# slimgroup/SetIntersectionProjection.jl

Hardware: AMD Instinct MI355X
Metric: PARSDMM iterations/sec (higher is better)
Workload: dtype f32

## Files before the change

### setintersectionprojection.jl_amd/csrc/engine.cpp

```cpp
#include "engine.h"
#include "comm.h"
#include "dist_dft.h"
#include "ext_proj.h"

#include <algorithm>
#include <chrono>
#include <cmath>
#include <cstdio>
#include <cstdlib>
#include <cstring>
#include <limits>
#include <map>
#include <mutex>
#include <thread>
#include <exception>

namespace sipx {

const LaunchObserver*& launch_observer() {
  static thread_local const LaunchObserver* obs = nullptr;
  return obs;
}

namespace {
EnvKnobs g_env_knobs;
}
const EnvKnobs& env_knobs() { return g_env_knobs; }
void refresh_env_knobs() {
  auto num = [](const char* name, long long dflt) { const char* e = std::getenv(name); return e ? std::atoll(e) : dflt; };
  EnvKnobs k;
  k.cds_march = (int)num("SIPX_CDS_MARCH", 1);
  k.cds_march_zchunk = num("SIPX_CDS_MARCH_ZCHUNK", 0);
  k.multi_zchunk = num("SIPX_MULTI_ZCHUNK", 0);
  k.rhs_march = (int)num("SIPX_RHS_MARCH", 1);
  k.rhs_march_zchunk = num("SIPX_RHS_MARCH_ZCHUNK", 0);
  k.q_plan = (int)num("SIPX_Q_PLAN", 1);
  k.mark_stride = (int)std::max<long long>(0, num("SIPX_MARK_STRIDE", 0));
  k.trace_searches = (int)num("SIPX_TRACE_SEARCHES", 0);
  k.trace_kernels = (int)num("SIPX_TRACE_KERNELS", 0);
  g_env_knobs = k;
}
long long*& alloc_tally() {
  static thread_local long long* t = nullptr;
  return t;
}

namespace {

struct TallyGuard {
  long long* prev;
  explicit TallyGuard(long long* t) : prev(alloc_tally()) { alloc_tally() = t; }
  ~TallyGuard() { alloc_tally() = prev; }
};

struct ObserverGuard {
  const LaunchObserver* prev;
  explicit ObserverGuard(const LaunchObserver* o) : prev(launch_observer()) { launch_observer() = o; }
  ~ObserverGuard() { launch_observer() = prev; }
};

constexpr int SLOTS = SET_SLOTS;

inline std::map<void*, long long>& tally_sizes() {
  static std::map<void*, long long> m;
  return m;
}
inline std::mutex& tally_mutex() {
  static std::mutex m;
  return m;
}
inline void tally_add(void* p, long long bytes) {
  if (long long* t = alloc_tally()) {
    *t += bytes;
    std::lock_guard<std::mutex> lk(tally_mutex());
    tally_sizes()[p] += bytes;
  }
}
inline void tally_release(void* p) {
  long long* t = alloc_tally();
  std::lock_guard<std::mutex> lk(tally_mutex());
  auto it = tally_sizes().find(p);
  if (it == tally_sizes().end()) return;
  if (t) *t -= it->second;
  tally_sizes().erase(it);
}
inline std::map<void*, size_t>& alloc_sizes() {
  static std::map<void*, size_t> m;
  return m;
}
template <typename T>
T* dalloc(size_t n, bool zero = true) {
  T* p = nullptr;
  if (n == 0) return p;
  SIPX_HIP(hipMalloc(&p, n * sizeof(T)));
  tally_add(p, (long long)(n * sizeof(T)));
  {
    std::lock_guard<std::mutex> lk(tally_mutex());
    alloc_sizes()[p] = n * sizeof(T);
  }
  if (zero) {
    SIPX_HIP(hipMemset(p, 0, n * sizeof(T)));
    SIPX_HIP(hipStreamSynchronize(nullptr));
  }
  return p;
}
struct SparseBlock {
  size_t total = 0;
  std::vector<std::pair<size_t, size_t>> maps;
  std::vector<hipMemGenericAllocationHandle_t> handles;
};
inline std::map<void*, SparseBlock>& sparse_registry() {
  static std::map<void*, SparseBlock> reg;
  return reg;
}
inline std::mutex& sparse_mutex() {
  static std::mutex m;
  return m;
}
constexpr size_t SPARSE_GRAN = 2ull << 20;
// ... 184 lines not shown
  long long Mtrue = 0, Mpad = 0;
  long long blk_rows[3] = {0, 0, 0};
  T plo = 0, phi = 0;
  bool ident = true, two_pass = false, is_dist = false, owned = true;
  bool in_sweep = false;
  T *y = nullptr, *l = nullptr, *dy = nullptr, *lh0 = nullptr, *y0 = nullptr, *s0 = nullptr, *l0 = nullptr;
  T *y2 = nullptr, *l2 = nullptr;
  int snap = -1;
  T *lb = nullptr, *ub = nullptr, *ata = nullptr;
  std::vector<void*> halo_allocs;
  int searches_done = 0;
  int ext_kind = 0;
  bool dist_ext = false;
  int owner_rank = 0;
  bool slab_ext = false, fan = false, slab_card = false, slab_dft = false;
  std::shared_ptr<DistDft<T>> ddft;
  int fan_owner = 0;
  bool fan_on_side = false;
  T* fanv = nullptr;
  hipEvent_t fan_ev = nullptr;
  ExtSpec spec;
  std::vector<T> host_basis;
  std::shared_ptr<ExtProj<T>> ext;
  ProjScalars<T>* ps = nullptr;
  ProjScalars<T>* psf = nullptr;
  std::vector<long long> ata_off;
  std::vector<T> host_lb, host_ub, host_ata;
  double sums[SLOTS] = {0};
  bool bb_valid = false;
  T last_rho = T(-1), last_gamma = T(-1);
  hipStream_t st = nullptr;
  hipEvent_t ev = nullptr;
  long long cbuf_len = 0;
  double* ptmp = nullptr;
  T *mpart = nullptr, *cbuf = nullptr;
};

}

template <typename T>
class Engine : public EngineBase {
 public:
  Engine(int ndim, const int64_t* n, const double* h, int device) : device_(device) {
    if (ndim != 2 && ndim != 3) throw std::runtime_error("ndim must be 2 or 3");
    SIPX_HIP(hipSetDevice(device));
    SIPX_HIP(hipStreamCreateWithFlags(&stream_, hipStreamNonBlocking));
    SIPX_HIP(hipEventCreateWithFlags(&ev_fork_, hipEventDisableTiming));
    SIPX_HIP(hipEventCreateWithFlags(&ev_fork2_, hipEventDisableTiming));
    {
      const char* e = std::getenv("SIPX_SERIAL_SETS");
      set_streams_ = !(e && e[0] == '1');
      const char* f = std::getenv("SIPX_CDS_FULL");
      cds_full_ = f && f[0] == '1';
      const char* k = std::getenv("SIPX_SET_STREAMS");
      if (k && std::atoi(k) > 0) { n_set_streams_ = std::atoi(k); set_streams_forced_ = true; }
    }
    ndim_ = ndim;
    for (int a = 0; a < 3; ++a) {
      G_.n[a] = a < ndim ? n[a] : 1;
      if (G_.n[a] < 1) throw std::runtime_error("grid size must be positive");
      ih_[a] = a < ndim ? T(1) / T(h[a]) : T(0);
    }
    if (ndim == 3 && G_.n[2] == 1) ndim_ = 2;
    G_.N = G_.n[0] * G_.n[1] * G_.n[2];
    if (G_.N <= (1ll << 22) && !set_streams_forced_ && !std::getenv("SIPX_SERIAL_SETS")) set_streams_ = false;
    G_.st[0] = 1;
    G_.st[1] = G_.n[0];
    G_.st[2] = G_.n[0] * G_.n[1];
    if (G_.N >= (1ll << 31)) throw std::runtime_error("grids of 2^31 points or more are not supported");
    G_.set_fast_div();
  }
  ~Engine() override {
    (void)hipSetDevice(device_);
    if (lane_thr_.joinable()) lane_thr_.join();
    if (lane_st_) { (void)hipStreamSynchronize(lane_st_); (void)hipStreamDestroy(lane_st_); }
    for (hipEvent_t e : {lane_fork_, lane_ev_}) if (e) (void)hipEventDestroy(e);
    dfree(lane_v_);
    if (fan_st_) { (void)hipStreamSynchronize(fan_st_); (void)hipStreamDestroy(fan_st_); }
    if (fan_fork_) (void)hipEventDestroy(fan_fork_);
    for (void* p : {(void*)fan_ptmp_, (void*)fan_mpart_, (void*)fan_c_}) dfree(p);
    if (loose_owned_) { dfree(loose_v_); dfree(loose_w_); }
    (void)hipStreamSynchronize(stream_);
    for (auto& s : sets_) free_set(s);
    for (void* p : {(void*)xr_base_[0], (void*)xr_base_[1], (void*)xr_base_[2], (void*)w_base_, (void*)rhs_, (void*)m_base_, (void*)r_base_, (void*)p_base_, (void*)p2_base_, (void*)Ap_, (void*)Q_, (void*)Q2_,
                    (void*)scr_v_, (void*)scr_c_, (void*)scr_i_, (void*)scr_w_, (void*)part_cg_, (void*)part_tmp_, (void*)part_sets_,
                    (void*)maxpart_, (void*)cg_dev_, (void*)gbuf_, (void*)stage_, (void*)sstage_, (void*)fbuf_, (void*)agree_buf_})
      dfree(p);
    comm_.reset();
    if (cstream_) (void)hipStreamDestroy(cstream_);
    for (auto e : ev_c_) if (e) (void)hipEventDestroy(e);
    if (ev_sums_) (void)hipEventDestroy(ev_sums_);
    for (hipEvent_t e : open_ev_) if (e) (void)hipEventDestroy(e);
    if (ev_cgb_) (void)hipEventDestroy(ev_cgb_);
    if (ticket_) (void)hipHostFree((void*)ticket_);
    if (cg_host_) (void)hipHostFree(cg_host_);
    if (hres_) (void)hipHostFree(hres_);
    if (sums_word_) (void)hipHostFree((void*)sums_word_);
    dfree(sums_ticket_);
    if (hlean_) (void)hipHostFree((void*)hlean_);
    if (hovf_) (void)hipHostFree((void*)hovf_);
    if (hverd_) (void)hipHostFree((void*)hverd_);
    for (auto e : ev_) (void)hipEventDestroy(e);
    for (auto e : stat_ev_) (void)hipEventDestroy(e);
    for (auto e : cg_ev_) if (e) (void)hipEventDestroy(e);
    for (hipStream_t q : pool_) if (q != stream_) (void)hipStreamDestroy(q);
    if (ev_fork_) (void)hipEventDestroy(ev_fork_);
    if (ev_fork2_) (void)hipEventDestroy(ev_fork2_);
    (void)hipStreamDestroy(stream_);
  }

  int add_set(const sipx_set_desc* d, const void* ata_R, const int64_t* ata_off, int d_i) override {
    if (finalized_) throw std::runtime_error("sipx_add_set after sipx_finalize");
    SetState<T> s;
    if (d->op == SIPX_OP_CSC) configure_custom(s, d);
    else configure_op(s, d->op);
    configure_proj(s, d);
    if (s.custom && !ata_R) throw std::runtime_error("a custom sparse operator needs its A'A in CDS (ata_R, ata_off)");
    if (s.custom && (s.comp || s.ext_kind))
      throw std::runtime_error("custom sparse operators: Minkowski components and library-backed projectors are not available");
    if (ata_R && s.comp) throw std::runtime_error("Minkowski sets use descriptor-generated AtA (pass ata_R = NULL)");
    if (ata_R) {
      if (d_i < 1 || d_i > 9) throw std::runtime_error("AtA band count out of range (1..9 bands per set)");
      s.ata_off.assign(ata_off, ata_off + d_i);
      s.host_ata.assign((const T*)ata_R, (const T*)ata_R + (size_t)G_.N * d_i);
    } else {
      s.ata_off = default_ata_offsets(s);
    }
    sets_.push_back(std::move(s));
    return (int)sets_.size() - 1;
  }

  int64_t set_rows(int set) override {
    if (set == (int)sets_.size() && !finalized_) return G_.N;
    if (set < 0 || set >= (int)sets_.size()) throw std::runtime_error("set index out of range");
    return sets_[set].Mtrue;
  }
  void num_terms(int* p, int* pp) override {
    if (p) *p = p_n_;
    if (pp) *pp = pp_n_;
  }
  void set_owned(const int32_t* owned) override {
    if (finalized_) throw std::runtime_error("sipx_set_owned must precede sipx_finalize");
    owned_.assign(owned, owned + sets_.size() + 1);
  }

  void set_decomp(int mode) override {
    if (finalized_) throw std::runtime_error("sipx_set_decomp must precede sipx_finalize");
    if (mode != SIPX_DECOMP_SETS && mode != SIPX_DECOMP_SLAB && mode != SIPX_DECOMP_SLAB_FULL) throw std::runtime_error("unknown decomposition");
    slab_req_ = mode != SIPX_DECOMP_SETS;
    slab_full_req_ = mode == SIPX_DECOMP_SLAB_FULL;
  }

  void set_comm(Comm* c) override {
    std::unique_ptr<Comm> hold(c);
    if (finalized_) throw std::runtime_error("the communicator must be attached before sipx_finalize");
    counting_ = c ? new CountingComm(hold.release()) : nullptr;
    comm_.reset(counting_);
  }
  void comm_info(int* nranks, int* rank, char* version, int version_len, int* decomposition) override {
    if (version && version_len > 0) version[0] = 0;
    if (nranks) *nranks = 1;
    if (rank) *rank = 0;
    if (decomposition) *decomposition = (finalized_ ? slab_ : (slab_req_ && comm_)) ? SIPX_DECOMP_SLAB : SIPX_DECOMP_SETS;
    if (comm_) comm_->info(nranks, rank, version, version_len > 0 ? (size_t)version_len : 0);
    else if (version && version_len > 0) std::snprintf(version, (size_t)version_len, "none");
  }
  void bind_device() override { SIPX_HIP(hipSetDevice(device_)); }
// ... 363 lines not shown
      if (sweep_plain_ && s.in_sweep) { s.y2 = halloc(s.Mpad); s.l2 = halloc(s.Mpad); }
      if (s.custom) upload_custom(s);
      if (s.slab_dft) {
        const long long nn[3] = {G_.n[0], G_.n[1], G_.n[2]};
        s.ddft = std::make_shared<DistDft<T>>(nn, r0_ / plane_, r1_ / plane_, chunk_ / plane_, comm_->world, comm_->rank, (double)s.spec.pmax, stream_);
      }
      if (s.ext_kind && !s.dist_ext && !s.slab_ext && !s.slab_dft && !(s.fan && s.fan_owner != comm_->rank)) {
        s.spec.lb = s.host_lb.empty() ? nullptr : s.host_lb.data();
        s.spec.ub = s.host_ub.empty() ? nullptr : s.host_ub.data();
        s.spec.basis = s.host_basis.empty() ? nullptr : s.host_basis.data();
        s.ext = std::make_shared<ExtProj<T>>(s.spec, stream_);
        if (s.ext_kind == EXT_HISTOGRAM) { s.host_lb.clear(); s.host_ub.clear(); }
        s.host_basis.clear();
        s.host_basis.shrink_to_fit();
      }
      if (s.fan) {
        s.fanv = (s.fan_owner == comm_->rank || !slab_local_) ? dalloc<T>(fullpad) : loose_alloc(Npad);
        SIPX_HIP(hipEventCreateWithFlags(&s.fan_ev, hipEventDisableTiming));
        if (s.fan_owner == comm_->rank && !fan_st_) {
          SIPX_HIP(hipStreamCreateWithFlags(&fan_st_, hipStreamNonBlocking));
          SIPX_HIP(hipEventCreateWithFlags(&fan_fork_, hipEventDisableTiming));
          fan_ptmp_ = dalloc<double>((size_t)(PREP_SLOTS + 2) * NB);
          fan_mpart_ = dalloc<T>(2 * NB);
          fan_c_ = dalloc<T>(fullpad);
        }
      }
      if (s.two_pass) {
        s.ps = dalloc<ProjScalars<T>>(1);
        s.psf = dalloc<ProjScalars<T>>(1);
        K<T>::ps_init(stream_, s.ps, scr_i_);
        K<T>::ps_init(stream_, s.psf, scr_i_);
      }
      if ((slab_ || search_batch_) && s.two_pass) {
        s.ptmp = dalloc<double>((size_t)(PREP_SLOTS + 2) * NB);
        s.mpart = dalloc<T>(2 * NB);
        s.cbuf_len = slab_local_ ? std::min<long long>(s.Mpad, std::max<long long>((long long)s.nblk_or1() * (whi_ - wlo_), hooks_.gcap + 64)) : s.Mpad;
        s.cbuf = dalloc<T>(s.cbuf_len);
      }
      const bool had_scratch = s.ptmp != nullptr;
      if (set_streams_ && !s.ext_kind && s.prox != PX_CARD) {
        if ((int)pool_.size() < n_set_streams_) {
          hipStream_t q = stream_;
          if (!pool_.empty()) SIPX_HIP(hipStreamCreateWithFlags(&q, hipStreamNonBlocking));
          pool_.push_back(q);
        }
        if (search_streams_) {
          while ((int)pool_.size() < n_set_streams_) {
            hipStream_t q2 = stream_;
            if (!pool_.empty()) SIPX_HIP(hipStreamCreateWithFlags(&q2, hipStreamNonBlocking));
            pool_.push_back(q2);
          }
          s.st = s.two_pass ? pool_[(size_t)(++search_next_) % pool_.size()] : pool_[0];
        } else {
          s.st = pool_[pool_next_++ % pool_.size()];
        }
        SIPX_HIP(hipEventCreateWithFlags(&s.ev, hipEventDisableTiming));
        if (s.two_pass && !had_scratch) {
          s.ptmp = dalloc<double>((size_t)(PREP_SLOTS + 2) * NB);
          s.mpart = dalloc<T>(2 * NB);
          s.cbuf = dalloc<T>(s.Mpad);
        }
      }
      if (s.prox == SIPX_PROJ_BOUNDS_VEC) {
        s.lb = dalloc<T>(s.Mpad); s.ub = dalloc<T>(s.Mpad);
        upload_rows(s, s.host_lb.data(), s.lb);
        upload_rows(s, s.host_ub.data(), s.ub);
      }
      if (warm && l0 && l0[i]) upload_rows_ranged(s, (const T*)l0[i], s.l);
      if (warm && y0 && y0[i]) upload_rows_ranged(s, (const T*)y0[i], s.y);
    }
    if (search_batch_) {
      int n2 = 0;
      for (auto& s : sets_) n2 += s.two_pass ? 1 : 0;
      fbuf_ = dalloc<T>((size_t)n2 * fast_hdr<T>());
      stage_ = dalloc<double>((size_t)n2 * (PREP_SLOTS + 1 + 2));
    }
    if (warm && x0) {
      const long long c0 = slab_local_ ? std::max<long long>(0, wlo_) : 0, c1 = slab_local_ ? std::min<long long>(Nx_, whi_) : Nx_;
      if (c1 > c0) SIPX_HIP(hipMemcpy(x_ + c0, (const T*)x0 + c0, (c1 - c0) * sizeof(T), hipMemcpyHostToDevice));
    }

    assemble_Q();
    if (q_fused_ && !stencil_q_ && !comm_ && cds_.march != 0) Q2_ = dalloc<T>((size_t)Nx_ * cds_.d);
    {
      const char* ln = std::getenv("SIPX_RANK_LANE");
      lane_set_ = -1;
      if (!comm_ && !mk_ && sweep_partial_ && !(ln && ln[0] == '0'))
        for (int i = 0; i < p_n_ && lane_set_ < 0; ++i) {
          const SetState<T>& s = sets_[i];
          if (s.owned && !s.in_sweep && !s.dist_ext && s.ident && !s.custom && s.ext && (s.ext_kind == EXT_RANK || s.ext_kind == EXT_NUCLEAR)) lane_set_ = i;
        }
      if (comm_ && slab_ && slab_loose_ && !mk_ && sweep_partial_ && !(ln && ln[0] == '0'))
        for (int i = 0; i < p_n_ && lane_set_ < 0; ++i) {
          const SetState<T>& s = sets_[i];
          if (s.owned && !s.in_sweep && s.slab_ext && s.ident && !s.custom && s.ext && (s.ext_kind == EXT_RANK || s.ext_kind == EXT_NUCLEAR)) lane_set_ = i;
        }
      if (lane_set_ >= 0) {
        const char* lp = std::getenv("SIPX_LANE_PRIORITY");
        int pr_least = 0, pr_greatest = 0;
        SIPX_HIP(hipDeviceGetStreamPriorityRange(&pr_least, &pr_greatest));
        if (lp && lp[0] == '0') SIPX_HIP(hipStreamCreateWithFlags(&lane_st_, hipStreamNonBlocking));
        else SIPX_HIP(hipStreamCreateWithPriority(&lane_st_, hipStreamNonBlocking, lp && lp[0] == 'l' ? pr_least : pr_greatest));
        SIPX_HIP(hipEventCreateWithFlags(&lane_fork_, hipEventDisableTiming));
        SIPX_HIP(hipEventCreateWithFlags(&lane_ev_, hipEventDisableTiming));
        if (slab_) lane_v_ = (slab_local_ && !loose_whole_) ? loose_alloc(Npad) : dalloc<T>((size_t)std::max<long long>(fullpad, sets_[lane_set_].Mpad));
        else lane_v_ = dalloc<T>((size_t)sets_[lane_set_].Mpad);
      }
    }
    } catch (const std::exception& ex) {
      if (!comm_ || comm_->world <= 1 || !agree_buf_) throw;
      alloc_err = ex.what();
    }
    if (comm_ && comm_->world > 1 && agree_buf_) {
      const double flag = alloc_err.empty() ? 0.0 : 1.0;
      double sum = flag;
      try {
        SIPX_HIP(hipMemcpy(agree_buf_, &flag, sizeof(double), hipMemcpyHostToDevice));
        comm_->allreduce_sum(agree_buf_, 1, SIPX_F64, stream_);
        SIPX_HIP(hipStreamSynchronize(stream_));
        SIPX_HIP(hipMemcpy(&sum, agree_buf_, sizeof(double), hipMemcpyDeviceToHost));
      } catch (const std::exception& ex) {
        throw std::runtime_error(std::string("sipx_finalize: the ranks could not agree on the outcome of their allocations (") + ex.what() + ")" +
                                 (alloc_err.empty() ? "" : "; this rank: " + alloc_err));
      }
      if (sum != 0.0)
        throw std::runtime_error("sipx_finalize failed on " + std::to_string((int)sum) + " of " + std::to_string(comm_->world) + " ranks while allocating" +
                                 (alloc_err.empty() ? std::string(" (not on this one)") : ": " + alloc_err));
    }
    finalized_ = true;

    initial_feasibility(feasibility_initial);
  }

  void reset(const void* m, const double* rho_ini, int n_rho, double gamma_ini, int zero_ini_guess, const void* x0,
             const void* const* l0, const void* const* y0, double* feasibility_initial) override {
    need_final();
    if (comm_) throw std::runtime_error("sipx_reset is not available for a rank of a sharded solve (build a new context)");
    SIPX_HIP(hipSetDevice(device_));
    if (lane_thr_.joinable()) lane_thr_.join();
    lane_err_ = nullptr;
    SIPX_HIP(hipStreamSynchronize(stream_));
    for (hipStream_t q : pool_) if (q && q != stream_) SIPX_HIP(hipStreamSynchronize(q));
    if (lane_st_) SIPX_HIP(hipStreamSynchronize(lane_st_));
    if (cstream_) SIPX_HIP(hipStreamSynchronize(cstream_));
    const long long N = G_.N;
    for (int k = 0; k < 3; ++k) dzero(xr_base_[k], stream_);
    dzero(p_base_, stream_); dzero(rhs_, stream_); dzero(r_base_, stream_); dzero(Ap_, stream_);
    dzero(p2_base_, stream_); dzero(w_base_, stream_); dzero(Q2_, stream_);
    dzero(part_cg_, stream_); dzero(part_tmp_, stream_); dzero(part_sets_, stream_); dzero(maxpart_, stream_);
    dzero(cg_dev_, stream_); dzero(sums_ticket_, stream_);
    dzero(fbuf_, stream_); dzero(stage_, stream_); dzero(sstage_, stream_); dzero(gbuf_, stream_);
    dzero(scr_v_, stream_); dzero(scr_c_, stream_); dzero(scr_w_, stream_);
    if (scr_i_) dzero(scr_i_, stream_);
    dzero(lane_v_, stream_);
    SIPX_HIP(hipMemcpyAsync(m_, m, N * sizeof(T), hipMemcpyHostToDevice, stream_));
    x_cur_ = 0; x_snap_ = -1;
    x_ = xr_[0]; xold_ = x_;
    if (n_rho == 1) std::fill(rho_.begin(), rho_.end(), (T)rho_ini[0]);
    else if (n_rho == p_n_) for (int i = 0; i < p_n_; ++i) rho_[i] = (T)rho_ini[i];
    else throw std::runtime_error("rho_ini must have 1 or p entries");
    T g0 = (T)gamma_ini;
    if (any_ncvx_) g0 = T(0.75);
    std::fill(gamma_.begin(), gamma_.end(), g0);
    const bool warm = !zero_ini_guess;
    for (int i = 0; i < p_n_; ++i) {
      SetState<T>& s = sets_[i];
      for (void* b : s.halo_allocs) dzero(b, stream_);
      dzero(s.lh0, stream_); dzero(s.s0, stream_);
      dzero(s.sbuf, stream_);
      dzero(s.ptmp, stream_); dzero(s.mpart, stream_); dzero(s.cbuf, stream_);
      s.snap = -1;
      s.searches_done = 0;
      std::fill(s.sums, s.sums + SLOTS, 0.0);
      s.bb_valid = false;
      s.last_rho = T(-1); s.last_gamma = T(-1);
      if (s.ps) K<T>::ps_init(stream_, s.ps, scr_i_);
      if (s.psf) K<T>::ps_init(stream_, s.psf, scr_i_);
      if (s.ext) { s.ext->set_stream(stream_); s.ext->reset(); }
      if (warm && l0 && l0[i]) upload_rows_ranged(s, (const T*)l0[i], s.l);
      if (warm && y0 && y0[i]) upload_rows_ranged(s, (const T*)y0[i], s.y);
    }
    if (warm && x0) SIPX_HIP(hipMemcpyAsync(x_, x0, Nx_ * sizeof(T), hipMemcpyHostToDevice, stream_));
    std::memset(cg_host_, 0, 2 * sizeof(CgState<T>));
    std::memset((void*)ticket_, 0xff, 64);
    std::memset(hres_, 0, sizeof(double) * (p_n_ + 1) * SLOTS);
    std::memset((void*)sums_word_, 0, 64);
    std::memset((void*)hlean_, 0, sizeof(int) * (p_n_ + 1));
    std::memset((void*)hovf_, 0, sizeof(int) * (p_n_ + 1));
    std::memset((void*)hverd_, 0, sizeof(unsigned) * (p_n_ + 1));
    sums_seq_ = 0; cg_seq_ = 0; spec_seq_ = 0;
    spec_searches_ = spec_fallbacks_ = spec_rounds_ = 0;
    batch_searches_ = batch_fallbacks_ = 0;
    head_done_ = false; rs_pending_ = false; sums_pending_ = false; defer_sums_ = false; merge_sums_ = false; merged_nslots_ = 0;
    q_pending_ = false; q_defer_ = false; rhs_fused_ = false; fuse_rhs_ = false; have_log_sums_ = false;
    obj_ss_ = evo_ss_ = xx_ss_ = 0;
    sums_flags_ = 0; word_sums_ = false;
    for (bool& v : open_valid_) v = false;
    mark_weight_[0] = mark_weight_[1] = 1.0;
    nmark_[0] = nmark_[1] = 0;
    mark_step_[0] = mark_step_[1] = 0;
    run_ = Run();
    assemble_Q();
    initial_feasibility(feasibility_initial);
  }

  void initial_feasibility(double* feasibility_initial) {
    feas_init_.assign(pp_n_, 0.0);
    for (int i = 0; i < pp_n_; ++i) {
      SetState<T>& s = sets_[i];
      if (s.dist_ext || s.slab_ext || s.slab_dft) {
        dist_feasibility(s, m_, part_sets_ + ((size_t)i * SLOTS + SL_FE2) * NB, i);
        continue;
      }
      if (s.fan) {
        SetArgs<T> a = set_args(s, rho_[i], gamma_[i], 0);
        a.x = m_;
        fan_feasibility(s, a, part_sets_ + ((size_t)i * SLOTS + SL_FE2) * NB);
        continue;
      }
      if (!s.owned) continue;
      if (slab_local_ && !s.two_pass && !s.ext_kind && !s.custom) {
        SetArgs<T> a = set_args(s, rho_[i], gamma_[i], 0);
        a.x = m_;
        K<T>::proj_dist_set(stream_, Gr_, a, 1, (const ProjScalars<T>*)nullptr, part_sets_ + ((size_t)i * SLOTS + SL_FE2) * NB);
        continue;
      }
      if (slab_ && !s.two_pass && comm_->rank != 0) continue;
      double* dst = part_sets_ + ((size_t)i * SLOTS + SL_FE2) * NB;
      const T* mm = s.comp == 2 ? w_ : m_;
      if (s.ext_kind) {
        SetArgs<T> a = set_args(s, rho_[i], gamma_[i], 0);
        a.x = mm;
        ext_feasibility(s, a, dst);
      } else if (s.custom) {
        K<T>::csr_spmv(stream_, s.Mtrue, s.d_rowptr, s.d_colidx, s.d_rval, mm, s.sbuf);
        if (s.two_pass) {
          SetArgs<T> a = set_args(s, rho_[i], gamma_[i], 0);
          a.x = s.sbuf;
          K<T>::proj_scalars_set(stream_, s.gm, a, 1, s.psf, part_tmp_, maxpart_, scr_c_, s.Mtrue);
          K<T>::proj_dist_set(stream_, s.gm, a, 1, s.psf, dst);
        } else {
          proj_dist_grid<T>(stream_, s.gm, 0, s.dir, s.Mpad, s.sbuf, s.prox, s.plo, s.phi, s.lb, s.ub, nullptr, dst);
        }
      } else if (s.two_pass) {
        SetArgs<T> a = set_args(s, rho_[i], gamma_[i], 0);
        a.x = mm;
        SampleCtl cf;
        cf.host_ovf = (int*)hovf_ + i;
        cf.compact_cap = scr_c_len_;
        K<T>::proj_scalars_set(stream_, Gr_, a, 1, s.psf, part_tmp_, maxpart_, scr_c_, s.Mtrue, cf, hooks());
        K<T>::proj_dist_set(stream_, Gr_, a, 1, s.psf, dst);
      } else {
        K<T>::fwd(stream_, G_, s.nblk, s.dir, s.ih, mm, scr_v_);
        proj_dist_grid<T>(stream_, G_, s.nblk, s.dir, s.Mpad, scr_v_, s.prox, s.plo, s.phi, s.lb, s.ub, nullptr, dst);
      }
    }
    reduce_set_sums(p_n_ * SLOTS);
    SIPX_HIP(hipStreamSynchronize(stream_));
    for (int i = 0; i < p_n_ && slab_; ++i)
      if (hovf_[i]) {
        hovf_[i] = 0;
        throw std::runtime_error("initial feasibility of set " + std::to_string(i) + ": the magnitudes inside the final bracket of the l1 search, gathered over all ranks, exceed the exchange segment of " +
                                 std::to_string(hooks_.gcap) + " values per rank (slab decomposition) -- use the set decomposition for this problem");
      }
    for (int i = 0; i < pp_n_; ++i) {
      if (!sets_[i].owned && !comm_) continue;
      feas_init_[i] = (double)feas_value(hres_[i * SLOTS + SL_FE2], hres_[i * SLOTS + SL_SS2]);
    }
    if (feasibility_initial)
      for (int i = 0; i < pp_n_; ++i) feasibility_initial[i] = feas_init_[i];
  }

  void rhs_compose(const double* rho) override {
    need_final();
    ObserverGuard og(observer());
    head_done_ = false;
    if (rs_pending_) {
      SIPX_HIP(hipStreamWaitEvent(stream_, ev_c_[1], 0));
      rs_pending_ = false;
    }
    if (mk_) {
      for (int half = 0; half < 2; ++half) {
        T* out = rhs_ + (long long)half * G_.N;
        int launched = 0;
        for (int pass = 0; pass < 2; ++pass) {
// ... 1258 lines not shown
      if (s.is_dist) {
        obj_ss_ = h[SL_OBJ]; evo_ss_ = h[SL_EVO]; xx_ss_ = h[SL_XX];
        if (mk_) { evo_ss_ = hres_[(size_t)p_n_ * SLOTS + SL_EVO]; xx_ss_ = hres_[(size_t)p_n_ * SLOTS + SL_XX]; }
        have_log_sums_ = true;
      }
    }
    if (all && !slab_dist_logs_) {
      const double* g = hres_ + (size_t)p_n_ * SLOTS;
      obj_ss_ = g[SL_OBJ]; evo_ss_ = g[SL_EVO]; xx_ss_ = g[SL_XX];
      have_log_sums_ = true;
    }
    if ((flags & SIPX_YL_FEAS) && feas) {
      for (int i = 0; i < pp_n_; ++i) {
        feas[i] = 0;
        if (!sets_[i].owned && !all) continue;
        const double* h = hres_ + (size_t)i * SLOTS;
        feas[i] = (sets_[i].two_pass || sets_[i].ext_kind) ? (double)feas_value(h[SL_FE2], h[SL_SS2])
                                                            : (double)feas_value(h[SL_FE], h[SL_SS]);
      }
    }
  }

  void log_scalars(double* obj, double* evol_x) override {
    need_final();
    ObserverGuard og(observer());
    if (!have_log_sums_) {
      K<T>::log3(stream_, G_.N, mk_ ? w_ : x_, m_, xold_, part_sets_);
      if (mk_) K<T>::log3(stream_, Nx_, x_, (const T*)nullptr, xold_, part_sets_ + (size_t)SLOTS * NB);
      K<T>::fin_sum(stream_, part_sets_, (mk_ ? 2 : 1) * SLOTS, nullptr, hres_);
      SIPX_HIP(hipStreamSynchronize(stream_));
      obj_ss_ = hres_[SL_OBJ]; evo_ss_ = hres_[SL_EVO]; xx_ss_ = hres_[SL_XX];
      if (mk_) { evo_ss_ = hres_[SLOTS + SL_EVO]; xx_ss_ = hres_[SLOTS + SL_XX]; }
    }
    const T nd = (T)std::sqrt(obj_ss_);
    *obj = (double)(T(0.5) * (nd * nd));
    *evol_x = (double)((T)std::sqrt(evo_ss_) / (T)std::sqrt(xx_ss_));
  }

  void adapt_rho_gamma(int adjust_rho, int adjust_gamma, double* rho_io, double* gamma_io) override {
    need_final();
    for (int i = 0; i < p_n_; ++i) {
      SetState<T>& s = sets_[i];
      if (!s.owned && !comm_) continue;
      if (!s.bb_valid)
        throw std::runtime_error("sipx_adapt_rho_gamma: call sipx_update_y_l with SIPX_YL_BB (or _FIRST) first");
      T rho = (T)rho_io[i], gamma = (T)gamma_io[i];
      const double* h = s.sums;
      bb_rule<T>((T)h[SL_HL], (T)std::sqrt(h[SL_HH]), (T)std::sqrt(h[SL_LH]), (T)std::sqrt(h[SL_DL]),
                 (T)std::sqrt(h[SL_GG]), (T)h[SL_GL], adjust_rho != 0, adjust_gamma != 0, rho, gamma);
      rho_io[i] = (double)rho;
      gamma_io[i] = (double)gamma;
    }
  }

  void q_update(const double* rho_new, const double* rho_old) override {
    need_final();
    ObserverGuard og(observer());
    if (stencil_q_) {
      stencil_weights(rho_new);
      return;
    }
    if (mk_) {
      std::vector<T> al(p_n_);
      for (int i = 0; i < p_n_; ++i) al[i] = rho_new[i] == rho_old[i] ? T(0) : (T)rho_new[i] - (T)rho_old[i];
      mk_q_update(al);
      return;
    }
    flush_q_pending();
    QArgs<T> a;
    a.nsets = 0;
    for (int i = 0; i < p_n_; ++i) {
      if (rho_new[i] == rho_old[i]) continue;
      push_qset(a, sets_[i], (T)rho_new[i] - (T)rho_old[i]);
    }
    if (q_defer_ && q_fused_ && cds_.march != 0 && !comm_ && a.nsets > 0) {
      bool generated = true;
      for (int k = 0; k < a.nsets; ++k) generated &= a.s[k].ata == nullptr;
      if (generated) {
        q_pending_args_ = a;
        q_pending_ = true;
        return;
      }
    }
    K<T>::q_update(stream_, G_, qr0_, qr1_, cds_, a, Q_);
  }
  void flush_q_pending() {
    if (!q_pending_) return;
    q_pending_ = false;
    K<T>::q_update(stream_, G_, qr0_, qr1_, cds_, q_pending_args_, Q_);
  }

  void warm_start_from(EngineBase* coarse_base) override {
    need_final();
    auto* c = dynamic_cast<Engine<T>*>(coarse_base);
    if (!c || !c->finalized_) throw std::runtime_error("warm start: the coarse context must be a finalized context of the same precision");
    if (c->device_ != device_) throw std::runtime_error("warm start: both levels must live on one device");
    if (c->p_n_ != p_n_ || c->ndim_ != ndim_ || mk_ || c->mk_) throw std::runtime_error("warm start: the two levels must hold the same sets");
    if ((comm_ != nullptr) != (c->comm_ != nullptr) || (comm_ && !(slab_ && c->slab_)))
      throw std::runtime_error("warm start between levels of a sharded solve needs both levels slab-decomposed (sipx_set_decomp)");
    long long nc[3], nf[3];
    for (int a = 0; a < 3; ++a) { nc[a] = c->G_.n[a]; nf[a] = G_.n[a]; }
    const long long Nc = c->G_.N, Nf = G_.N;
    const long long cpad = c->comm_ ? c->chunk_ * c->comm_->world : Nc;
    int nbmax = 1;
    for (auto& st : c->sets_) nbmax = std::max(nbmax, st.nblk_or1());
    T* whole = c->slab_ ? dalloc<T>((size_t)nbmax * cpad, false) : nullptr;
    const int dt = dtype_code();
    const long long f0 = slab_local_ ? std::max<long long>(0, wlo_) : 0, f1 = slab_local_ ? std::min<long long>(Nf, whi_) : Nf;
    auto complete = [&](const T* src, int nb) -> const T* {
      if (!c->slab_) return src;
      const long long nloc = c->r1_ - c->r0_;
      for (int q = 0; q < nb; ++q) {
        T* w = whole + (long long)q * cpad;
        if (nloc > 0) SIPX_HIP(hipMemcpyAsync(w + c->r0_, src + (long long)q * Nc + c->r0_, nloc * sizeof(T), hipMemcpyDeviceToDevice, stream_));
        c->comm_->allgather(w, (size_t)c->chunk_, dt, stream_);
      }
      return whole;
    };
    const long long cstride = c->slab_ ? cpad : Nc;
    SIPX_HIP(hipStreamSynchronize(c->stream_));
    resample_nn_padded<T>(stream_, nc, nf, nc, nf, f0, f1, complete(c->x_, 1), x_);
    for (int i = 0; i < p_n_; ++i) {
      SetState<T>&f = sets_[i], &g = c->sets_[i];
      if (f.custom || g.custom || f.nblk != g.nblk) throw std::runtime_error("warm start: operator kinds differ between the levels");
      for (int q = 0; q < f.nblk; ++q)
        if (f.dir[q] != g.dir[q]) throw std::runtime_error("warm start: operator kinds differ between the levels");
      if (!f.owned || !g.owned) continue;
      for (int which = 0; which < 2; ++which) {
        const T* src = complete(which ? g.y : g.l, g.nblk_or1());
        T* dst = which ? f.y : f.l;
        if (f.nblk >= 2) {
          for (int q = 0; q < f.nblk; ++q)
            resample_nn_rows<T>(stream_, nc, nf, f.nblk, f.dir, q, cstride, f0, f1, src, dst + (long long)q * Nf);
        } else {
          long long cc[3], cf[3];
          for (int a = 0; a < 3; ++a) { cc[a] = nc[a]; cf[a] = nf[a]; }
          if (f.nblk == 1) { cc[f.dir[0]] -= 1; cf[f.dir[0]] -= 1; }
          resample_nn_padded<T>(stream_, nc, nf, cc, cf, f0, f1, src, dst);
        }
      }
    }
    SIPX_HIP(hipStreamSynchronize(stream_));
    dfree(whole);
  }

  void gather_slabs(bool want_x, const std::vector<char>& want_l, const std::vector<char>& want_y) {
    const int dt = dtype_code();
    if (want_x) comm_->allgather(x_, (size_t)chunk_, dt, stream_);
    for (int i = 0; i < p_n_; ++i)
      for (int which = 0; which < 2; ++which) {
        if (!(which ? want_y[i] : want_l[i])) continue;
        T* arr = which ? sets_[i].y : sets_[i].l;
        const int nb = sets_[i].nblk > 0 ? sets_[i].nblk : 1;
        for (int q = 0; q < nb; ++q) {
          T* blk = arr + (long long)q * G_.N;
          if (r1_ > r0_) SIPX_HIP(hipMemcpyAsync(scr_v_ + r0_, blk + r0_, (r1_ - r0_) * sizeof(T), hipMemcpyDeviceToDevice, stream_));
          comm_->allgather(scr_v_, (size_t)chunk_, dt, stream_);
          SIPX_HIP(hipMemcpyAsync(blk, scr_v_, G_.N * sizeof(T), hipMemcpyDeviceToDevice, stream_));
        }
      }
  }

  void download_sparse(void* x, void* const* l, void* const* y) {
    const int dt = dtype_code();
    const long long N = G_.N, Npad = chunk_ * comm_->world, nloc = r1_ - r0_;
    int nbmax = 1;
    for (auto& s : sets_) nbmax = std::max(nbmax, s.nblk_or1());
    T* exch = dalloc<T>((size_t)Npad);
    T* whole = dalloc<T>((size_t)nbmax * N);
    auto complete = [&](const T* src) {
      if (nloc > 0) SIPX_HIP(hipMemcpyAsync(exch + r0_, src + r0_, nloc * sizeof(T), hipMemcpyDeviceToDevice, stream_));
      comm_->allgather(exch, (size_t)chunk_, dt, stream_);
// ... 286 lines not shown
    for (int a = 0; a < 3; ++a) H = std::max<long long>(H, G_.st[a]);
    H = (H + 3) / 4 * 4;
    T* dxb = dalloc<T>(G_.N + 2 * H);
    T* dvb = dalloc<T>(s.Mpad + H);
    T *dx = dxb + H, *dv = dvb + H;
    if (!adjoint) {
      SIPX_HIP(hipMemcpy(dx, x, G_.N * sizeof(T), hipMemcpyHostToDevice));
      K<T>::fwd(stream_, G_, s.nblk, s.dir, s.ih, dx, dv);
      download_rows(s, dv, (T*)out);
    } else {
      upload_rows(s, (const T*)x, dv);
      K<T>::adj(stream_, G_, s.nblk, s.dir, s.ih, dv, dx);
      SIPX_HIP(hipStreamSynchronize(stream_));
      SIPX_HIP(hipMemcpy(out, dx, G_.N * sizeof(T), hipMemcpyDeviceToHost));
    }
    dfree(dxb);
    dfree(dvb);
  }

  void project(const sipx_set_desc* d, void* v, int64_t len) override {
    SIPX_HIP(hipSetDevice(device_));
    Grid g1;
    g1.n[0] = len; g1.n[1] = 1; g1.n[2] = 1; g1.N = len; g1.st[0] = 1; g1.st[1] = len; g1.st[2] = len;
    T* dv = dalloc<T>(len);
    T* dc = dalloc<T>(len);
    T *lb = nullptr, *ub = nullptr;
    double* part = dalloc<double>((size_t)(PREP_SLOTS + 2) * NB);
    T* mp = dalloc<T>(2 * NB);
    ProjScalars<T>* ps = dalloc<ProjScalars<T>>(1);
    SIPX_HIP(hipMemcpy(dv, v, len * sizeof(T), hipMemcpyHostToDevice));
    const int prox = d->proj;
    const T plo = (T)d->pmin, phi = (T)d->pmax;
    if (prox == SIPX_PROJ_BOUNDS_VEC && d->mode == SIPX_MODE_WHOLE && d->transform == SIPX_TRANSFORM_NONE) {
      if (!d->lb || !d->ub) throw std::runtime_error("per-element bounds need lb and ub");
      lb = dalloc<T>(len); ub = dalloc<T>(len);
      SIPX_HIP(hipMemcpy(lb, d->lb, len * sizeof(T), hipMemcpyHostToDevice));
      SIPX_HIP(hipMemcpy(ub, d->ub, len * sizeof(T), hipMemcpyHostToDevice));
    }
    if (prox == SIPX_PROJ_L1 && !(d->pmax > 0)) throw std::runtime_error("Radius of L1 ball is negative");
    if (d->mode != SIPX_MODE_WHOLE || d->transform != SIPX_TRANSFORM_NONE || prox == SIPX_PROJ_L1_DFT || prox >= SIPX_PROJ_RANK) {
      if (len != G_.N) throw std::runtime_error("this projector / application mode needs a vector of the grid size");
      SetState<T> st;
      configure_op(st, SIPX_OP_IDENTITY);
      configure_proj(st, d);
      if (st.ext_kind) {
        st.spec.lb = st.host_lb.empty() ? nullptr : st.host_lb.data();
        st.spec.ub = st.host_ub.empty() ? nullptr : st.host_ub.data();
        st.spec.basis = st.host_basis.empty() ? nullptr : st.host_basis.data();
        ExtProj<T> ext(st.spec, stream_);
        ext.project(dv, false, part, mp, dc);
      } else {
        lb = dalloc<T>(len); ub = dalloc<T>(len);
        SIPX_HIP(hipMemcpy(lb, st.host_lb.data(), len * sizeof(T), hipMemcpyHostToDevice));
        SIPX_HIP(hipMemcpy(ub, st.host_ub.data(), len * sizeof(T), hipMemcpyHostToDevice));
        proj_apply_grid<T>(stream_, g1, 0, nullptr, len, dv, st.prox, st.plo, st.phi, lb, ub, nullptr);
      }
      SIPX_HIP(hipStreamSynchronize(stream_));
      SIPX_HIP(hipMemcpy(v, dv, len * sizeof(T), hipMemcpyDeviceToHost));
      for (void* q : {(void*)dv, (void*)dc, (void*)part, (void*)mp, (void*)ps, (void*)lb, (void*)ub})
        if (q) dfree(q);
      return;
    }
    const bool two = prox == SIPX_PROJ_L1 || prox == SIPX_PROJ_L2 || prox == SIPX_PROJ_ANNULUS || prox == SIPX_PROJ_CARDINALITY;
    long long* di = prox == SIPX_PROJ_CARDINALITY ? dalloc<long long>(len) : nullptr;
    if (two) {
      K<T>::ps_init(stream_, ps, di);
      K<T>::proj_scalars_arr(stream_, len, dv, prox, plo, phi, ps, part, mp, dc, len);
    }
    proj_apply_grid<T>(stream_, g1, 0, nullptr, len, dv, prox, prox == SIPX_PROJ_BOUNDS_VEC ? T(0) : plo, phi, lb, ub, two ? ps : nullptr);
    SIPX_HIP(hipStreamSynchronize(stream_));
    SIPX_HIP(hipMemcpy(v, dv, len * sizeof(T), hipMemcpyDeviceToHost));
    for (void* q : {(void*)dv, (void*)dc, (void*)lb, (void*)ub, (void*)part, (void*)mp, (void*)ps, (void*)di})
      dfree(q);
  }

  void get_Q(void* Q, int64_t* offsets, int* d) override {
    need_final();
    SIPX_HIP(hipStreamSynchronize(stream_));
    if (d) *d = cds_.d;
    if (offsets) for (int b = 0; b < cds_.d; ++b) offsets[b] = cds_.off[b];
    if (Q && stencil_q_) throw std::runtime_error("stencil Q mode stores no bands (use sipx_apply_Q)");
    if (Q && comm_ && comm_->world > 1) throw std::runtime_error("a sharded context maintains its slab of Q only");
    flush_q_pending();
    if (Q && cds_.sym) {
      K<T>::mirror_bands(stream_, Nx_, cds_, Q_);
      SIPX_HIP(hipStreamSynchronize(stream_));
    }
    if (Q) SIPX_HIP(hipMemcpy(Q, Q_, (size_t)Nx_ * cds_.d * sizeof(T), hipMemcpyDeviceToHost));
  }

  void apply_Q(const void* x, void* y) override {
    need_final();
    if (comm_ && comm_->world > 1) throw std::runtime_error("a sharded context maintains its slab of Q only");
    SIPX_HIP(hipStreamSynchronize(stream_));
    SIPX_HIP(hipMemcpy(p_, x, Nx_ * sizeof(T), hipMemcpyHostToDevice));
    flush_q_pending();
    if (stencil_q_) K<T>::sq_spmv(stream_, G_, sq_, p_, Ap_);
    else K<T>::spmv(stream_, G_, Nx_, Q_, cds_, p_, Ap_);
    SIPX_HIP(hipStreamSynchronize(stream_));
    SIPX_HIP(hipMemcpy(y, Ap_, Nx_ * sizeof(T), hipMemcpyDeviceToHost));
  }

  double time_spmv(int reps) override {
    need_final();
    flush_q_pending();
    hipEvent_t a, b;
    SIPX_HIP(hipEventCreate(&a));
    SIPX_HIP(hipEventCreate(&b));
    auto one = [&]() {
      if (stencil_q_) K<T>::sq_spmv(stream_, G_, sq_, x_, Ap_);
      else K<T>::spmv(stream_, G_, Nx_, Q_, cds_, x_, Ap_);
    };
    one();
    SIPX_HIP(hipEventRecord(a, stream_));
    for (int k = 0; k < reps; ++k) one();
    SIPX_HIP(hipEventRecord(b, stream_));
    SIPX_HIP(hipEventSynchronize(b));
    float ms = 0;
    SIPX_HIP(hipEventElapsedTime(&ms, a, b));
    (void)hipEventDestroy(a);
    (void)hipEventDestroy(b);
    return (double)ms / reps;
  }

  void kernel_stats(int enable, int64_t* launches, double* total_ms) override {
    need_final();
    std::vector<KAgg> agg = aggregate_samples();
    const KAgg& a = stencil_q_ ? agg[KID_SQ_DOT] : agg[KID_CDS_DOT];
    if (launches) *launches = a.launches;
    if (total_ms) *total_ms = a.ms;
    start_stats(enable);
  }
  const char* kernel_stats_json(int enable) override {
    need_final();
    const bool peek = enable < 0;
    std::vector<KAgg> agg = peek ? std::vector<KAgg>(KID_COUNT) : aggregate_samples();
    std::string& o = stats_json_;
    o = "{\"mode\": " + std::to_string(stats_mode_) + ", \"event_pair_overhead_ms\": " + std::to_string(stat_pair_ms_) + ", \"kernels\": [";
    bool first = true;
    char buf[512];
    for (int k = 0; k < KID_COUNT; ++k) {
      if (!agg[k].launches) continue;
      const bool gated = gated_kernel(k);
      std::snprintf(buf, sizeof buf,
                    "%s{\"name\": \"%s\", \"launches\": %lld, \"noop_launches\": %lld, \"total_ms\": %.6f, \"bytes_survey\": %.0f, "
                    "\"bytes_moved\": %.0f, \"gated\": %s, \"inclusive\": %s}",
                    first ? "" : ", ", kernel_name(k), (long long)agg[k].launches, (long long)agg[k].noops, agg[k].ms, agg[k].bytes_survey,
                    agg[k].bytes_moved,
                    gated ? "true" : "false", k == KID_EXT ? "true" : "false");
      o += buf;
      first = false;
    }
    o += "], \"slab_searches\": {\"speculative_exchange\": " + std::to_string(spec_searches_) + ", \"fallbacks\": " +
         std::to_string(spec_fallbacks_) + ", \"refinement_rounds\": " + std::to_string(spec_rounds_) + "}";
    o += std::string(", \"sparse_arrays\": ") + (slab_local_ ? "true" : "false");
    {
      std::string loc, fan;
      for (int i = 0; i < p_n_; ++i) {
        if (sets_[i].slab_ext || sets_[i].slab_card || sets_[i].slab_dft) loc += (loc.empty() ? "" : ", ") + std::to_string(i);
        if (sets_[i].fan) fan += (fan.empty() ? "" : ", ") + std::to_string(i);
      }
      if (counting_)
        o += ", \"collectives\": {\"allreduce\": " + std::to_string(counting_->n_allreduce) + ", \"allreduce_with_halo\": " + std::to_string(counting_->n_grouped) +
             ", \"allgather\": " + std::to_string(counting_->n_allgather) + ", \"reduce_scatter\": " + std::to_string(counting_->n_reduce_scatter) +
             ", \"halo\": " + std::to_string(counting_->n_halo) + ", \"scatter_gather\": " + std::to_string(counting_->n_fan) +
             ", \"alltoall\": " + std::to_string(counting_->n_alltoall) + "}";
      o += ", \"slab_loose\": {\"slab_local_sets\": [" + loc + "], \"gathered_sets\": [" + fan + "], \"fan_exchanges\": " + std::to_string(fan_exchanges_) + "}";
    }
    {
      std::string t = selftest_;
      for (auto& ch : t) if (ch == '"' || ch == '\\' || (unsigned char)ch < 32) ch = ' ';
      o += ", \"comm_selftest\": \"" + t + "\"";
    }
    o += ", \"lane_set\": " + std::to_string(lane_set_);
    o += ", \"batched_searches\": {\"searches\": " + std::to_string(batch_searches_) + ", \"fallbacks\": " + std::to_string(batch_fallbacks_) + "}";
    long long rc[6] = {0, 0, 0, 0, 0, 0};
    for (const auto& st : sets_) {
      if (!st.ext || st.ext_kind != EXT_RANK) continue;
      long long c[6];
      st.ext->route_counts(c);
      for (int q = 0; q < 6; ++q) rc[q] += c[q];
    }
    o += ", \"rank_route\": {\"calls\": " + std::to_string(rc[0]) + ", \"warm_started_subspace\": " + std::to_string(rc[1]) +
         ", \"full_decomposition\": " + std::to_string(rc[2]) + ", \"products_with_gram\": " + std::to_string(rc[3]) +
         ", \"float32_loops\": " + std::to_string(rc[4]) + ", \"float32_gave_up\": " + std::to_string(rc[5]) + "}}";
    if (!peek) start_stats(enable);
    return o.c_str();
  }
  double stat_pair_overhead_ms() const { return stat_pair_ms_; }

  void debug_proj(int set, int which, double* o) override {
    need_final();
    for (int k = 0; k < 16; ++k) o[k] = 0;
    if (set < 0 || set >= p_n_) throw std::runtime_error("set index out of range");
    const ProjScalars<T>* d = (which & 1) ? sets_[set].psf : sets_[set].ps;
    if (!d) return;
    ProjScalars<T> h;
    SIPX_HIP(hipStreamSynchronize(stream_));
    SIPX_HIP(hipMemcpy(&h, d, sizeof(h), hipMemcpyDeviceToHost));
    o[0] = h.need; o[1] = h.theta; o[2] = h.theta_prev; o[3] = h.hw; o[4] = h.spec_lo; o[5] = h.spec_hi; o[6] = h.lo;
    o[7] = h.hi; o[8] = h.asum; o[9] = h.vmax; o[10] = h.dbg[0]; o[11] = h.dbg[1]; o[12] = h.dbg[2]; o[13] = h.dbg[3];
    o[14] = h.refine;
    o[15] = h.lean + 2 * h.dbg_sampled;
    if (which & 2) { o[4] = h.samp_theta; o[5] = h.samp_lo; o[6] = h.samp_hi; o[7] = h.samp_c; }
  }

  void* stream() override { return (void*)stream_; }
  void* dev_rhs() override { return rhs_; }
  void* dev_x() override { return x_; }
  void get_rhs(void* out) override {
    need_final();
    if (slab_local_ && comm_->world > 1) throw std::runtime_error("a slab-decomposed context holds its planes of rhs only");
    SIPX_HIP(hipStreamSynchronize(stream_));
    SIPX_HIP(hipMemcpy(out, rhs_, Nx_ * sizeof(T), hipMemcpyDeviceToHost));
  }

 private:
  struct KSample { int kid; double bytes_survey, bytes_moved; };
  struct KAgg { long long launches = 0, noops = 0; double ms = 0, bytes_survey = 0, bytes_moved = 0; };
  hipEvent_t stat_event(size_t i) {
    while (stat_ev_.size() <= i) {
      hipEvent_t e;
      SIPX_HIP(hipEventCreate(&e));
      stat_ev_.push_back(e);
    }
    return stat_ev_[i];
  }
  static void obs_begin(void* user, int kid, hipStream_t s, double bytes_survey, double bytes_moved) {
    auto* e = static_cast<Engine<T>*>(user);
    if (e->stats_mode_ == 0 || (e->stats_mode_ == 1 && kid != KID_CDS_DOT && kid != KID_SQ_DOT)) return;
    const size_t i = e->samples_.size();
    e->samples_.push_back(KSample{kid, bytes_survey, bytes_moved});
    e->open_.push_back(i);
    SIPX_HIP(hipEventRecord(e->stat_event(2 * i), s));
  }
  static void obs_end(void* user, int kid, hipStream_t s) {
    auto* e = static_cast<Engine<T>*>(user);
    if (e->stats_mode_ == 0 || (e->stats_mode_ == 1 && kid != KID_CDS_DOT && kid != KID_SQ_DOT)) return;
    if (e->open_.empty()) return;
    const size_t i = e->open_.back();
    e->open_.pop_back();
    if (i < e->samples_.size()) SIPX_HIP(hipEventRecord(e->stat_event(2 * i + 1), s));
  }
  void drop_samples_from(size_t n) {
    if (n < samples_.size()) samples_.resize(n);
    open_.clear();
  }
  void sync_all_streams() {
    SIPX_HIP(hipStreamSynchronize(stream_));
    for (hipStream_t q : pool_) if (q != stream_) SIPX_HIP(hipStreamSynchronize(q));
    if (cstream_) SIPX_HIP(hipStreamSynchronize(cstream_));
  }
  static bool gated_kernel(int k) {
    return k == KID_PASS_FIRST || k == KID_PASS_LEAN || k == KID_PASS_PROBE || k == KID_PASS_COMPACT || k == KID_SAMPLE ||
           k == KID_DECIDE || k == KID_CDS_FUSED || k == KID_CG_XR || k == KID_CG_P || k == KID_SLOT_SUMS;
  }
  std::vector<KAgg> aggregate_samples() {
// ... 269 lines not shown
  }

  int q_col(long long off) const {
    for (int b = 0; b < cds_.d; ++b)
      if (cds_.off[b] == off) return b;
    throw std::runtime_error("attempted to update a diagonal in A in CDS storage that does not exist. A and B need "
                             "to have the same nonzero diagonals");
  }

  void plan_Q_offsets() {
    std::vector<long long> seen;
    auto see = [&](long long o) {
      if (std::find(seen.begin(), seen.end(), o) == seen.end()) seen.push_back(o);
    };
    for (auto& s : sets_) {
      if (s.ata_off.size() > 999) throw std::runtime_error("more than 999 bands in one set");
      for (long long o : s.ata_off) see(o);
      see(0);
    }
    if ((int)seen.size() > MAXD) throw std::runtime_error("Q has more bands than this build supports");
    cds_.d = (int)seen.size();
    for (int b = 0; b < cds_.d; ++b) cds_.off[b] = seen[b];
    bool ok = !cds_full_;
    for (int b = 0; b < cds_.d && ok; ++b) {
      cds_.partner[b] = b;
      if (cds_.off[b] >= 0) continue;
      int pb = -1;
      for (int c = 0; c < cds_.d; ++c)
        if (cds_.off[c] == -cds_.off[b]) pb = c;
      if (pb < 1) ok = false;
      else cds_.partner[b] = pb;
    }
    for (auto& s : sets_) ok = ok && (s.host_ata.empty() || explicit_bands_symmetric(s));
    cds_.sym = ok ? 1 : 0;
    cds_.march = 0;
    if (cds_.sym && cds_.d == 7 && ndim_ == 3 && !mk_) {
      const long long s1 = G_.st[1], s2 = G_.st[2];
      const long long o1[7] = {0, -1, 1, -s1, s1, -s2, s2}, o2[7] = {0, -s2, -s1, -1, 1, s1, s2};
      bool m1 = true, m2 = true;
      for (int b = 0; b < 7; ++b) { m1 = m1 && cds_.off[b] == o1[b]; m2 = m2 && cds_.off[b] == o2[b]; }
      cds_.march = m1 ? 1 : (m2 ? 2 : 0);
      const long long want[4] = {0, 1, s1, s2};
      for (int q = 0; q < 4; ++q)
        for (int b = 0; b < 7; ++b)
          if (cds_.off[b] == want[q]) cds_.mb[q] = b;
      for (int a = 0; a < 3; ++a) cds_.gn[a] = G_.n[a];
    }
  }

  bool explicit_bands_symmetric(const SetState<T>& s) const {
    const long long N = G_.N;
    for (size_t b = 0; b < s.ata_off.size(); ++b) {
      const long long o = s.ata_off[b];
      if (o >= 0) continue;
      long long pb = -1;
      for (size_t c = 0; c < s.ata_off.size(); ++c)
        if (s.ata_off[c] == -o) pb = (long long)c;
      if (pb < 0) return false;
      const T* lo = s.host_ata.data() + b * (size_t)N;
      const T* up = s.host_ata.data() + (size_t)pb * (size_t)N;
      for (long long r = -o; r < N; ++r)
        if (std::memcmp(&lo[r], &up[r + o], sizeof(T)) != 0) return false;
    }
    return true;
  }

  void stencil_weights(const double* rho) {
    double w0 = 0, w[3] = {0, 0, 0};
    sq_.mask = 0;
    for (int i = 0; i < p_n_; ++i) {
      const SetState<T>& s = sets_[i];
      const double r = (double)(T)rho[i];
      if (s.nblk == 0) w0 += r;
      for (int q = 0; q < s.nblk; ++q) {
        w[s.dir[q]] += r * (double)(T)(s.ih[q] * s.ih[q]);
        sq_.mask |= 1 << s.dir[q];
      }
    }
    sq_.w0 = (T)w0;
    for (int d = 0; d < 3; ++d) sq_.w[d] = (T)w[d];
  }

  void assemble_Q() {
    if (stencil_q_) {
      for (auto& s : sets_)
        if (s.ata) throw std::runtime_error("stencil Q mode needs descriptor-generated AtA for every set (pass ata_R = NULL)");
      std::vector<double> r(rho_.begin(), rho_.end());
      stencil_weights(r.data());
      return;
    }
    if (Q_) {
      dzero(Q_, stream_);
    } else if (slab_local_) {
      std::vector<std::pair<size_t, size_t>> rg;
      long long maxoff = 0;
      for (int b = 0; b < cds_.d; ++b) maxoff = std::max<long long>(maxoff, std::llabs(cds_.off[b]));
      for (int b = 0; b < cds_.d; ++b) {
        const long long lo = std::max<long long>(0, (long long)b * Nx_ + (r1_ > r0_ ? r0_ : 0) - maxoff - 64);
        const long long hi = std::min<long long>((long long)Nx_ * cds_.d, (long long)b * Nx_ + std::max(qr1_, qr0_) + 64);
        if (hi > lo) rg.push_back({(size_t)lo * sizeof(T), (size_t)hi * sizeof(T)});
      }
      Q_ = (T*)sparse_alloc_bytes((size_t)Nx_ * cds_.d * sizeof(T), rg, device_);
    } else {
      Q_ = dalloc<T>((size_t)Nx_ * cds_.d);
    }
    if (mk_) {
      std::vector<T> al(rho_.begin(), rho_.end());
      mk_q_update(al);
      return;
    }
    QArgs<T> a;
    a.nsets = 0;
    for (int i = 0; i < p_n_; ++i) push_qset(a, sets_[i], rho_[i]);
    K<T>::q_update(stream_, G_, qr0_, qr1_, cds_, a, Q_);
  }

  void mk_q_update(const std::vector<T>& alpha) {
    MkArgs<T> a;
    a.nsets = 0;
    for (int i = 0; i < p_n_; ++i) {
      if (alpha[i] == T(0)) continue;
      const SetState<T>& s = sets_[i];
      for (long long o : s.ata_off) (void)q_col(o);
      MkSet<T>& m = a.s[a.nsets++];
      m.alpha = alpha[i];
      m.nblk = s.nblk;
      m.comp = s.comp;
      for (int k = 0; k < 3; ++k) { m.dir[k] = s.dir[k]; m.ih[k] = s.ih[k]; }
      if (a.nsets == MAX_SETS) {
        K<T>::q_update_mk(stream_, G_, cds_, a, Q_);
        a.nsets = 0;
      }
    }
    K<T>::q_update_mk(stream_, G_, cds_, a, Q_);
  }

  void push_qset(QArgs<T>& a, const SetState<T>& s, T alpha) {
    if (s.ata_off.size() > 9) throw std::runtime_error("more than 9 bands in one set's AtA are not supported");
    for (long long o : s.ata_off) (void)q_col(o);
    if (a.nsets == MAX_SETS) {
      K<T>::q_update(stream_, G_, qr0_, qr1_, cds_, a, Q_);
      a.nsets = 0;
    }
    QSet<T>& q = a.s[a.nsets++];
    q.alpha = alpha;
    q.ata = s.ata;
    q.nblk = s.nblk;
    for (int k = 0; k < 3; ++k) { q.dir[k] = s.dir[k]; q.ih[k] = s.ih[k]; }
    q.nband = (int)s.ata_off.size();
    for (int k = 0; k < q.nband; ++k) q.off[k] = s.ata_off[k];
  }

  SetArgs<T> set_args(const SetState<T>& s, T rho, T gamma, int flags) const {
    SetArgs<T> a;
    a.y = s.y; a.l = s.l; a.dy = s.dy; a.lh0 = s.lh0; a.s0 = s.s0;
    a.y0 = s.snap == 0 ? s.y : s.y0;
    a.l0 = s.snap == 0 ? s.l : s.l0;
    a.yo = s.y; a.lo = s.l;
    a.v = scr_v_;
    a.x = x_; a.m = m_; a.xold = xold_; a.lb = s.lb; a.ub = s.ub;
    a.nblk = s.nblk;
    for (int q = 0; q < 3; ++q) { a.dir[q] = s.dir[q]; a.ih[q] = s.ih[q]; }
    a.rho = rho;
    a.rho1 = T(1) / rho;
    a.gamma = gamma;
    a.prox = s.prox;
    a.plo = s.plo; a.phi = s.phi;
    a.ps = s.ps;
    a.flags = flags;
    a.vsrc = 0;
    return a;
  }

  void dist_feasibility(SetState<T>& s, const T* src, double* dst, int set = 0) {
    const long long nloc = r1_ - r0_;
    if (nloc > 0) {
      SIPX_HIP(hipMemcpyAsync(loose_v_ + r0_, src + r0_, nloc * sizeof(T), hipMemcpyDeviceToDevice, stream_));
      SIPX_HIP(hipMemcpyAsync(loose_w_ + r0_, src + r0_, nloc * sizeof(T), hipMemcpyDeviceToDevice, stream_));
      if (!s.slab_dft) s.ext->project(loose_v_ + r0_, true, part_tmp_, maxpart_, scr_c_);
    }
    if (s.slab_dft) s.ddft->project(loose_v_ + r0_, true, comm_.get(), &hooks_, part_tmp_, maxpart_, scr_c_, scr_c_len_, (int*)hovf_ + set);
    ext_dist2<T>(stream_, nloc, loose_v_ + r0_, loose_w_ + r0_, dst);
  }

  void fan_collect(SetState<T>& s, const SetArgs<T>& a, int v_is_s, T* buf) {
    if (r1_ > r0_) SIPX_HIP(hipMemsetAsync(buf + r0_, 0, (size_t)(r1_ - r0_) * sizeof(T), stream_));
    SetArgs<T> b = a;
    b.v = buf;
    K<T>::store_v(stream_, Gr_, b, v_is_s, buf);
    comm_->gather(buf, (size_t)chunk_, dtype_code(), s.fan_owner, stream_);
    ++fan_exchanges_;
  }
  void fan_project_owner(SetState<T>& s, bool feas, T* buf, hipStream_t q, double* ptmp, T* mpart, T* cbuf) {
    ObsScope obs(KID_EXT, q, 0.0);
    if (s.ext_kind) {
      s.ext->set_stream(q);
      s.ext->project(buf, feas, ptmp, mpart, cbuf);
    } else {
      ProjScalars<T>* ps = feas ? s.psf : s.ps;
      K<T>::proj_scalars_arr(q, G_.N, buf, s.prox, s.plo, s.phi, ps, ptmp, mpart, cbuf, s.Mtrue);
      proj_apply_grid<T>(q, G_, s.nblk, s.dir, G_.N, buf, s.prox, s.plo, s.phi, (const T*)nullptr, (const T*)nullptr, ps);
    }
  }
  void fan_begin(SetState<T>& s, const SetArgs<T>& a) {
    fan_collect(s, a, 0, s.fanv);
    if (comm_->rank != s.fan_owner) return;
    hipStream_t q = (fan_st_ && stats_mode_ != 2 && fan_overlap_) ? fan_st_ : stream_;
    if (q != stream_) {
      SIPX_HIP(hipEventRecord(fan_fork_, stream_));
      SIPX_HIP(hipStreamWaitEvent(q, fan_fork_, 0));
    }
    fan_project_owner(s, false, s.fanv, q, fan_ptmp_, fan_mpart_, fan_c_);
    if (q != stream_) SIPX_HIP(hipEventRecord(s.fan_ev, q));
    s.fan_on_side = q != stream_;
  }
  void fan_return(SetState<T>& s) {
    const int dt = dtype_code();
    T* buf = s.fanv;
    if (s.fan_on_side) { SIPX_HIP(hipStreamWaitEvent(stream_, s.fan_ev, 0)); s.fan_on_side = false; }
    comm_->scatter(buf, (size_t)chunk_, dt, s.fan_owner, stream_);
    ++fan_exchanges_;
    if (!s.ident && r1_ > r0_ && (prev_ >= 0 || next_ >= 0))
      comm_->halo_exchange(buf + r0_, buf + r0_ - plane_, prev_, buf + r1_ - plane_, buf + r1_, next_, (size_t)plane_, dt, stream_);
  }
// ... 216 lines not shown
  std::vector<T> rho_, gamma_;
  std::vector<double> feas_init_;
  T *x_base_ = nullptr, *p_base_ = nullptr, *m_base_ = nullptr, *r_base_ = nullptr, *p2_base_ = nullptr, *p2_ = nullptr;
  bool cg_fused_ = false;
  long long halo_ = 0;
  T *x_ = nullptr, *xold_ = nullptr, *rhs_ = nullptr, *m_ = nullptr, *r_ = nullptr, *p_ = nullptr, *Ap_ = nullptr;
  T *Q_ = nullptr, *scr_v_ = nullptr, *scr_c_ = nullptr, *maxpart_ = nullptr;
  long long* scr_i_ = nullptr;
  long long scr_c_len_ = 0;
  T* scr_w_ = nullptr;
  T *loose_v_ = nullptr, *loose_w_ = nullptr;
  bool loose_owned_ = false, loose_whole_ = false;
  bool need_idx_ = false, need_ext_ = false;
  CdsArgs cds_;
  bool cds_full_ = false;
  bool set_streams_ = true;
  hipEvent_t ev_fork_ = nullptr, ev_fork2_ = nullptr;
  std::vector<hipStream_t> pool_;
  bool set_streams_forced_ = false, search_streams_ = false;
  int search_next_ = 0;
  int n_set_streams_ = 2, pool_next_ = 0;
  bool mk_ = false;
  long long Nx_ = 0;
  T *w_base_ = nullptr, *w_ = nullptr;
  StencilQ<T> sq_{};
  bool stencil_q_ = false;
  double *part_cg_ = nullptr, *part_tmp_ = nullptr, *part_sets_ = nullptr;
  CgState<T>*cg_dev_ = nullptr, *cg_host_ = nullptr;
  double* hres_ = nullptr;
  volatile unsigned long long* sums_word_ = nullptr;
  unsigned* sums_ticket_ = nullptr;
  unsigned long long sums_seq_ = 0;
  bool sums_by_word_ = false, word_sums_ = false;
  volatile int* hlean_ = nullptr;
  volatile int* hovf_ = nullptr;
  volatile unsigned* hverd_ = nullptr;
  unsigned spec_seq_ = 0;
  long long spec_searches_ = 0, spec_fallbacks_ = 0, spec_rounds_ = 0;
  bool spec_exchange_ = true;
  int lane_set_ = -1;
  hipStream_t lane_st_ = nullptr;
  hipEvent_t lane_fork_ = nullptr, lane_ev_ = nullptr;
  T* lane_v_ = nullptr;
  std::thread lane_thr_;
  std::exception_ptr lane_err_;
  long long lane_sample_ = -1;
  SetArgs<T> lane_args_;
  bool sweep_partial_ = false, has_loose_ = false;
  bool pass_multi_ = false;
  bool sweep_plain_ = false;
  bool feas_sample_ = true;
  bool search_batch_ = false;
  long long batch_searches_ = 0, batch_fallbacks_ = 0;
  bool spec_batch_ = true;
  bool slab_lean_multi_ = true;
  T* fbuf_ = nullptr;
  long long l1_sample_runs_ = 0;
  bool l1_sample_ = true;
  bool yl_multi_ = true;
  bool x0_mode_ = false;
  T *xr_base_[3] = {nullptr, nullptr, nullptr}, *xr_[3] = {nullptr, nullptr, nullptr};
  int x_cur_ = 0, x_snap_ = -1;
  bool fuse_rhs_ = false;
  bool rhs_fused_ = false;
  std::vector<hipEvent_t> ev_;
  hipEvent_t open_ev_[4] = {nullptr, nullptr, nullptr, nullptr};
  bool open_valid_[4] = {false, false, false, false};
  int mark_step_[2] = {0, 0};
  double mark_weight_[2] = {1.0, 1.0};
  int nmark_[2] = {0, 0};
  int mark_sec_[2][MAXMARK];
  hipEvent_t sums_event_ = nullptr;
  std::unique_ptr<Comm> comm_;
  CountingComm* counting_ = nullptr;
  long long plane_ = 0, chunk_ = 0, r0_ = 0, r1_ = 0, qr0_ = 0, qr1_ = 0;
  int prev_ = -1, next_ = -1;
  hipStream_t cstream_ = nullptr;
  hipEvent_t ev_c_[2] = {nullptr, nullptr};
  bool rs_pending_ = false;
  double* dres_ = nullptr;
  hipEvent_t ev_sums_ = nullptr, ev_cgb_ = nullptr;
  bool sums_pending_ = false, defer_sums_ = false;
  bool q_fused_ = false, q_pending_ = false, q_defer_ = false;
  QArgs<T> q_pending_args_;
  T* Q2_ = nullptr;
  long long dev_bytes_ = 0;
  bool slab_dist_logs_ = false;
  bool lean_multi_ = false;
  bool head_done_ = false;
  bool merge_sums_ = false;
  int merged_nslots_ = 0;
  bool resid_ahead_ = true;
  int sums_flags_ = 0;
  volatile unsigned long long* ticket_ = nullptr;
  unsigned cg_seq_ = 0;
  bool slab_req_ = false, slab_ = false;
  hipStream_t fan_st_ = nullptr;
  hipEvent_t fan_fork_ = nullptr;
  double* fan_ptmp_ = nullptr;
  T *fan_mpart_ = nullptr, *fan_c_ = nullptr;
  long long fan_exchanges_ = 0;
  bool fan_overlap_ = true;
  bool slab_loose_ = false;
  bool slab_full_req_ = false, slab_local_ = false;
  std::string selftest_ = "none", mapped_why_;
  double* agree_buf_ = nullptr;
  bool selftest_mapped_failed_ = false, selftest_alltoall_failed_ = false;
  std::string a2a_why_;
  long long wlo_ = 0, whi_ = 0;
  Grid Gr_, Gyl_;
  ChainHooks hooks_;
  T* gbuf_ = nullptr;
  double *stage_ = nullptr, *sstage_ = nullptr;
  const ChainHooks* hooks() const { return slab_ ? &hooks_ : nullptr; }
  double obj_ss_ = 0, evo_ss_ = 0, xx_ss_ = 0;
  bool have_log_sums_ = false;
  hipEvent_t cg_ev_[2] = {nullptr, nullptr};
  std::vector<hipEvent_t> stat_ev_;
  std::vector<KSample> samples_;
  std::vector<size_t> open_;
  int stats_mode_ = 0;
  LaunchObserver obs_{this, &Engine<T>::obs_begin, &Engine<T>::obs_end};
  std::string stats_json_;
  double stat_pair_ms_ = 0;
};

EngineBase* make_engine(int dtype, int ndim, const int64_t* n, const double* h, int device) {
  int count = 0;
  if (hipGetDeviceCount(&count) != hipSuccess || count <= 0)
    throw std::runtime_error("libsipx: no HIP device visible -- this engine has no CPU fallback");
  if (device < 0 || device >= count) throw std::runtime_error("libsipx: device index out of range");
  if (dtype == SIPX_F32) return new Engine<float>(ndim, n, h, device);
  if (dtype == SIPX_F64) return new Engine<double>(ndim, n, h, device);
  throw std::runtime_error("dtype must be SIPX_F32 or SIPX_F64");
}

template <typename T>
static void cds_spmv_T(int64_t N, int d, const void* R, const int64_t* off, const void* x, void* y) {
  if (d < 1 || d > MAXD) throw std::runtime_error("cds_spmv: band count out of range");
  long long H = 4;
  for (int b = 0; b < d; ++b) H = std::max<long long>(H, std::llabs((long long)off[b]));
  H = (H + 3) / 4 * 4;
  T* dR = dalloc<T>((size_t)N * d, false);
  T* dxb = dalloc<T>(N + 2 * H);
  T* dx = dxb + H;
  T* dy = dalloc<T>(N);
  SIPX_HIP(hipMemcpy(dR, R, (size_t)N * d * sizeof(T), hipMemcpyHostToDevice));
  SIPX_HIP(hipMemcpy(dx, x, N * sizeof(T), hipMemcpyHostToDevice));
  CdsArgs a;
  a.d = d;
  for (int b = 0; b < d; ++b) a.off[b] = off[b];
  Grid g;
  g.n[0] = N; g.n[1] = 1; g.n[2] = 1; g.N = N; g.st[0] = 1; g.st[1] = N; g.st[2] = N;
  K<T>::spmv(nullptr, g, N, dR, a, dx, dy);
  SIPX_HIP(hipDeviceSynchronize());
  SIPX_HIP(hipMemcpy(y, dy, N * sizeof(T), hipMemcpyDeviceToHost));
  dfree(dR); dfree(dxb); dfree(dy);
}

template <typename T>
static void resample_T(int ndim, const int64_t* nc, const int64_t* nf, const void* in, void* out) {
  long long c[3] = {1, 1, 1}, f[3] = {1, 1, 1};
  for (int q = 0; q < ndim && q < 3; ++q) { c[q] = nc[q]; f[q] = nf[q]; }
  const long long Nc = c[0] * c[1] * c[2], Nf = f[0] * f[1] * f[2];
  if (Nc < 1 || Nf < 1) throw std::runtime_error("resample: empty array");
  T* di = dalloc<T>(Nc, false);
// ... 52 lines not shown
```

### setintersectionprojection.jl_amd/csrc/kernels_cds.hip

```cpp
#include <cstdlib>
#include <stdexcept>
#include <string>

#include "sipx_device.h"
#define SIPX_CG_GRID launch_blocks(3)
#ifndef SIPX_F64_VEC
#define SIPX_F64_VEC 2
#endif

namespace sipx {

template <typename T, int V>
struct LoadStored {
  const T* __restrict__ x;
  __device__ __forceinline__ Vec<T, V> operator()(long long c) const { return ldv_u<T, V>(x + c); }
};
template <typename T, int V>
struct LoadFused {
  const T* __restrict__ r;
  const T* __restrict__ p;
  T beta;
  __device__ __forceinline__ Vec<T, V> operator()(long long c) const {
    const Vec<T, V> rv = ldv_u<T, V>(r + c), pv = ldv_u<T, V>(p + c);
    Vec<T, V> o;
// ... 64 lines not shown
      for (int k = 0; k < V; ++k) o.v[k] = s[k];
      stv_nt<T, V>(y + r, o);
    } else if (MODE == 1) {
      const Vec<T, V> pv = ldv<T, V>(x + r);
      Vec<T, V> o;
#pragma unroll
      for (int k = 0; k < V; ++k) {
        o.v[k] = s[k];
        acc0 += (double)pv.v[k] * (double)s[k];
      }
      stv_nt<T, V>(y + r, o);
    } else {
      const Vec<T, V> bv = ldv<T, V>(b + r);
      const Vec<T, V> xv = ldv<T, V>(x + r);
      Vec<T, V> o;
#pragma unroll
      for (int k = 0; k < V; ++k) {
        o.v[k] = bv.v[k] - s[k];
        acc0 += (double)o.v[k] * (double)o.v[k];
        acc1 += (double)bv.v[k] * (double)bv.v[k];
      }
      stv<T, V>(y + r, o);
      if (pout) stv<T, V>(pout + r, o);
      if (xold) stv<T, V>(xold + r, xv);
    }
  }
  if (MODE == 1) {
    double acc[1] = {acc0};
    block_reduce_store<1>(acc, partials, 0);
  } else if (MODE == 2) {
    double acc[2] = {acc0, acc1};
    block_reduce_store<2>(acc, partials, 0);
  }
}

constexpr int march_role(int ord, int b) {
  constexpr int o1[7] = {0, 1, 2, 3, 4, 5, 6}, o2[7] = {0, 5, 3, 1, 2, 4, 6};
  return ord == 1 ? o1[b] : o2[b];
}
template <typename T>
__device__ __forceinline__ T ata_value(const Grid& G, int nblk, const int* dir, const T* ihs, long long o, const Coord& c) {
  T val = (nblk == 0 && o == 0) ? T(1) : T(0);
  for (int q = 0; q < nblk; ++q) {
    const int d = dir[q];
    const T ih = ihs[q], nih = -ih;
    const int cc = coord_of(c, d);
    const long long st = G.st[d];
    if (o == 0) {
      if (cc > 0) val = val + ih * ih;
      if (cc < G.n[d] - 1) val = val + nih * nih;
    } else if (o == st) {
      if (cc < G.n[d] - 1) val = val + nih * ih;
    } else if (o == -st) {
      if (cc > 0) val = val + ih * nih;
    }
  }
  return val;
}

constexpr int QP_MAXB = 9, QP_MAXT = 8, QP_TAB = 160;
struct QPlanTerm {
  int kind;
  int nblk;
  int dir[3];
  int tab;
};
template <typename T>
struct QPlan {
  int nbands;
  int col[QP_MAXB], nterms[QP_MAXB];
  QPlanTerm t[QP_MAXB][QP_MAXT];
  int ntab;
  T tab[QP_TAB];
};

template <typename T>
struct QUpd {
  QPlan<T> plan;
  int pb[4];
  T* qn[4];
  Grid G;
};
struct NoExtra {};
template <typename T>
__device__ __forceinline__ T q_upd_val(const QUpd<T>& u, const T* __restrict__ tab, int role, const Coord& c, T qv) {
  const int b = u.pb[role];
  if (b < 0) return qv;
  const int cx = c.i == 0 ? 0 : (c.i == (int)u.G.n[0] - 1 ? 2 : 1), cy = c.j == 0 ? 0 : (c.j == (int)u.G.n[1] - 1 ? 2 : 1),
            cz = c.k == 0 ? 0 : (c.k == (int)u.G.n[2] - 1 ? 2 : 1);
  for (int ti = 0; ti < u.plan.nterms[b]; ++ti) {
    const QPlanTerm& t = u.plan.t[b][ti];
    if (t.kind == 0) {
      qv = qv + tab[t.tab];
    } else if (t.kind == 1) {
      int idx = 0, m3 = 1;
      for (int q = 0; q < t.nblk; ++q) {
        const int d = t.dir[q];
        idx += (d == 0 ? cx : (d == 1 ? cy : cz)) * m3;
        m3 *= 3;
      }
      qv = qv + tab[t.tab + idx];
    } else {
      const int d = t.dir[0], cl = d == 0 ? cx : (d == 1 ? cy : cz);
      qv = qv + (cl != (t.kind == 2 ? 2 : 0) ? tab[t.tab] : tab[t.tab + 1]);
    }
  }
  return qv;
}
template <typename T>
__device__ __forceinline__ T q_upd_val(const NoExtra&, const T*, int, const Coord&, T qv) { return qv; }
template <typename T>
__device__ __forceinline__ void load_plan_tab(const QUpd<T>& u, T* tab) {
  for (int i = threadIdx.x; i < u.plan.ntab; i += blockDim.x) tab[i] = u.plan.tab[i];
}
template <typename T>
__device__ __forceinline__ void load_plan_tab(const NoExtra&, T*) {}
template <typename T>
__device__ __forceinline__ const Grid& extra_grid(const QUpd<T>& u) { return u.G; }
__device__ __forceinline__ Grid extra_grid(const NoExtra&) { return Grid{}; }
template <typename T, int V>
__device__ __forceinline__ void store_bands(const QUpd<T>& u, long long r, const Vec<T, V>& r0, const Vec<T, V>& r1, const Vec<T, V>& r2,
                                            const Vec<T, V>& r3) {
  stv<T, V>(u.qn[0] + r, r0);
  stv<T, V>(u.qn[1] + r, r1);
  stv<T, V>(u.qn[2] + r, r2);
  stv<T, V>(u.qn[3] + r, r3);
}
template <typename T, int V>
__device__ __forceinline__ void store_bands(const NoExtra&, long long, const Vec<T, V>&, const Vec<T, V>&, const Vec<T, V>&, const Vec<T, V>&) {}
__device__ __forceinline__ void publish_ticket(unsigned long long* ticket, unsigned seq, int iter, int done);
constexpr int MARCH_NT = 512;
template <typename T, int V, int ORD, int MODE, typename X>
__global__ __launch_bounds__(MARCH_NT) void k_cds_march(long long n1, long long n2, long long n3, long long z0, long long z1, const T* __restrict__ R0,
                                                        const T* __restrict__ R1, const T* __restrict__ R2, const T* __restrict__ R3,
                                                        const T* __restrict__ x, T* __restrict__ y, const T* __restrict__ b,
                                                        T* __restrict__ pout, T* __restrict__ xold, double* __restrict__ partials,
                                                        const int* __restrict__ done, int lgLX, int tiles_x, int tiles_y, int zchunk,
                                                        long long items, CgState<T>* __restrict__ st, CgState<T>* __restrict__ host,
                                                        unsigned long long* ticket, X extra) {
  constexpr bool UPD = MODE == 4;
  if (MODE == 1 && *done) return;
  T beta = T(0);
  if (MODE == 3) {
    if (st->done) return;
    const double ss = block_sum_partials_n<MARCH_NT>(partials + NB);
    const T rr = (T)ss;
    const T res = (T)sqrt(ss) / st->nr0;
    const bool conv = res <= st->tol;
    beta = rr / st->gamma;
    if (blockIdx.x == 0 && threadIdx.x == 0) {
      st->ss = ss;
      st->res_last = res;
      if (conv) { st->flag = 0; st->done = 1; } else { st->beta = beta; }
      st->rr = rr;
      *host = *st;
      publish_ticket(ticket, st->seq, st->iters, conv ? 1 : 0);
    }
    if (conv) return;
  }
  auto ldx = [&](long long at) -> Vec<T, V> {
    Vec<T, V> v = ldv<T, V>(x + at);
    if (MODE == 3) {
      const Vec<T, V> pv = ldv<T, V>(b + at);
#pragma unroll
      for (int k = 0; k < V; ++k) v.v[k] = v.v[k] + beta * pv.v[k];
    }
    return v;
  };
  auto ldx1 = [&](long long at) -> T { return MODE == 3 ? x[at] + beta * b[at] : x[at]; };
  __shared__ T sx[2][V][MARCH_NT], sr[2][V][MARCH_NT];
  __shared__ T qtab[UPD ? QP_TAB : 1];
  if (UPD) {
    load_plan_tab<T>(extra, qtab);
    __syncthreads();
  }
  const int tid = threadIdx.x, LX = 1 << lgLX, tx = tid & (LX - 1), ty = tid >> lgLX, TY = MARCH_NT >> lgLX;
  const long long st1 = n1, st2 = n1 * n2, N = st2 * n3;
  const long long tiles = (long long)tiles_x * tiles_y;
  double acc0 = 0, acc1 = 0;
  for (long long item = blockIdx.x; item < items; item += gridDim.x) {
    const long long zc = item / tiles, tile = item - zc * tiles;
    const int tile_y = (int)(tile / tiles_x), tile_x = (int)(tile - (long long)tile_y * tiles_x);
    const long long i0 = ((long long)tile_x * LX + tx) * V, j = (long long)tile_y * TY + ty;
    const bool active = i0 < n1 && j < n2;
    const long long k0 = z0 + zc * zchunk, k1 = (k0 + zchunk < z1) ? k0 + zchunk : z1;
    const unsigned go = active ? (unsigned)(i0 + st1 * j) : 0u;
    __syncthreads();
    Vec<T, V> xm = zerov<T, V>(), x0 = zerov<T, V>(), rzm = zerov<T, V>();
    if (active) {
      xm = ldx(st2 * (k0 - 1) + go);
      x0 = ldx(st2 * k0 + go);
      if (k0 > 0) {
        rzm = ldv<T, V>(R3 + st2 * (k0 - 1) + go);
        if (UPD) {
#pragma unroll
          for (int k = 0; k < V; ++k) rzm.v[k] = q_upd_val<T>(extra, qtab, 3, Coord{(int)(i0 + k), (int)j, (int)(k0 - 1)}, rzm.v[k]);
        }
      }
    }
    for (long long kz = k0; kz < k1; ++kz) {
      const int par = (int)(kz & 1);
      const long long pz = st2 * kz;
      Vec<T, V> xp = zerov<T, V>(), r0 = xp, r1 = xp, r2 = xp, r3 = xp, bv = xp;
      if (active) {
        xp = ldx(pz + st2 + go);
        r0 = ldv_nt<T, V>(R0 + pz + go);
        r1 = ldv_nt<T, V>(R1 + pz + go);
        r2 = ldv_nt<T, V>(R2 + pz + go);
        r3 = ldv_nt<T, V>(R3 + pz + go);
        if (MODE == 2 || MODE == 4) bv = ldv<T, V>(b + pz + go);
        if (UPD) {
#pragma unroll
          for (int k = 0; k < V; ++k) {
            const Coord ck{(int)(i0 + k), (int)j, (int)kz};
            r0.v[k] = q_upd_val<T>(extra, qtab, 0, ck, r0.v[k]);
            r1.v[k] = q_upd_val<T>(extra, qtab, 1, ck, r1.v[k]);
            r2.v[k] = q_upd_val<T>(extra, qtab, 2, ck, r2.v[k]);
            r3.v[k] = q_upd_val<T>(extra, qtab, 3, ck, r3.v[k]);
          }
        }
      }
#pragma unroll
      for (int k = 0; k < V; ++k) { sx[par][k][tid] = x0.v[k]; sr[par][k][tid] = r2.v[k]; }
      T xl = __shfl_up(x0.v[V - 1], 1, 64), xr = __shfl_down(x0.v[0], 1, 64), rl = __shfl_up(r1.v[V - 1], 1, 64);
      const long long r = pz + go;
      if (active) {
        if (tx == 0 || (tid & 63) == 0) {
          xl = ldx1(r - 1);
          rl = r > 0 ? R1[r - 1] : T(0);
          if (UPD && r > 0) rl = q_upd_val<T>(extra, qtab, 1, coords(extra_grid(extra), r - 1), rl);
        }
        if (tx == LX - 1 || (tid & 63) == 63) xr = ldx1(r + V);
      }
      __syncthreads();
      if (active) {
        Vec<T, V> xu = zerov<T, V>(), xd = xu, ru = xu;
        if (ty > 0) {
#pragma unroll
          for (int k = 0; k < V; ++k) { xu.v[k] = sx[par][k][tid - LX]; ru.v[k] = sr[par][k][tid - LX]; }
        } else {
          xu = ldx(r - st1);
          if (r - st1 >= 0) {
            ru = ldv<T, V>(R2 + r - st1);
            if (UPD) {
#pragma unroll
              for (int k = 0; k < V; ++k) ru.v[k] = q_upd_val<T>(extra, qtab, 2, coords(extra_grid(extra), r - st1 + k), ru.v[k]);
            }
          }
        }
        if (ty < TY - 1 && j + 1 < n2) {
#pragma unroll
          for (int k = 0; k < V; ++k) xd.v[k] = sx[par][k][tid + LX];
        } else {
          xd = ldx(r + st1);
        }
        Vec<T, V> o4;
#pragma unroll
        for (int k = 0; k < V; ++k) {
          const long long rr = r + k;
          const T rv[7] = {r0.v[k], k == 0 ? rl : r1.v[k - 1], r1.v[k], ru.v[k], r2.v[k], rzm.v[k], r3.v[k]};
          const T xv[7] = {x0.v[k], k == 0 ? xl : x0.v[k - 1], k == V - 1 ? xr : x0.v[k + 1], xu.v[k], xd.v[k], xm.v[k], xp.v[k]};
          const long long co[7] = {0, -1, 1, -st1, st1, -st2, st2};
          T acc = T(0);
#pragma unroll
          for (int q = 0; q < 7; ++q) {
            const int role = march_role(ORD, q);
            const T t = acc + rv[role] * xv[role];
            const long long c = rr + co[role];
            acc = (c >= 0 && c < N) ? t : acc;
          }
          o4.v[k] = acc;
        }
        if (MODE == 0) {
          stv_nt<T, V>(y + r, o4);
        } else if (MODE == 1 || MODE == 3) {
#pragma unroll
          for (int k = 0; k < V; ++k) acc0 += (double)x0.v[k] * (double)o4.v[k];
          stv_nt<T, V>(y + r, o4);
          if (MODE == 3) stv<T, V>(pout + r, x0);
        } else {
          Vec<T, V> o;
#pragma unroll
          for (int k = 0; k < V; ++k) {
            o.v[k] = bv.v[k] - o4.v[k];
            acc0 += (double)o.v[k] * (double)o.v[k];
            acc1 += (double)bv.v[k] * (double)bv.v[k];
          }
          stv<T, V>(y + r, o);
          if (pout) stv<T, V>(pout + r, o);
          if (xold) stv<T, V>(xold + r, x0);
          if (UPD) store_bands<T, V>(extra, r, r0, r1, r2, r3);
        }
      }
      xm = x0; x0 = xp; rzm = r3;
    }
  }
  if (MODE != 0) {
    __shared__ double sm[2][MARCH_NT / 64];
    const double v0 = wave_sum(acc0), v1 = wave_sum(acc1);
    __syncthreads();
    if ((tid & 63) == 0) { sm[0][tid >> 6] = v0; sm[1][tid >> 6] = v1; }
    __syncthreads();
    if (tid < ((MODE == 2 || MODE == 4) ? 2 : 1)) {
      double s = 0;
#pragma unroll
      for (int i = 0; i < MARCH_NT / 64; ++i) s += sm[tid][i];
      double* row = partials + (long long)tid * NB;
      row[blockIdx.x] = s;
      for (int jj = blockIdx.x + gridDim.x; jj < NB; jj += gridDim.x) row[jj] = 0.0;
    }
  }
}

template <typename T, int MODE>
static bool try_march(hipStream_t s, long long N, long long r0, long long r1, const T* R, const CdsArgs& a, const T* x, T* y, const T* b,
                      T* pout, T* xold, double* partials, const int* done, CgState<T>* st = nullptr, CgState<T>* host = nullptr,
                      unsigned long long* ticket = nullptr, const QUpd<T>* upd = nullptr) {
  const int sw = env_knobs().cds_march;
  const long long zc_env = env_knobs().cds_march_zchunk;
  if (sw == 0 || !a.march || !a.sym || a.d != 7) return false;
  constexpr int V = sizeof(T) == 8 ? 2 : 4;
  const long long n1 = a.gn[0], n2 = a.gn[1], n3 = a.gn[2], st2 = n1 * n2;
  if (n1 % V != 0 || n1 * n2 * n3 != N || r0 % st2 != 0 || r1 % st2 != 0 || r1 <= r0) return false;
  const long long nvx = n1 / V;
  int lg = 0;
  while ((1 << lg) < nvx && lg < 6) ++lg;
  const int LX = 1 << lg, TY = MARCH_NT / LX;
  const int tiles_x = (int)((nvx + LX - 1) / LX), tiles_y = (int)((n2 + TY - 1) / TY);
  const long long tiles = (long long)tiles_x * tiles_y, planes = (r1 - r0) / st2;
  long long zchunk = planes * tiles / 2048;
  if (zchunk < 16) zchunk = 16;
  if (sw == 2 && zc_env > 0) zchunk = zc_env;
  if (zchunk > planes) zchunk = planes;
  const long long nchunks = (planes + zchunk - 1) / zchunk, items = tiles * nchunks;
  if (items < 384 && sw != 2) return false;
  const int grid = (int)(items < NB ? items : NB);
  const T *R0 = R + (long long)a.mb[0] * N, *R1 = R + (long long)a.mb[1] * N, *R2 = R + (long long)a.mb[2] * N, *R3 = R + (long long)a.mb[3] * N;
#define SIPX_MARCH(ORD, XT, XV)                                                                                                      \
  hipLaunchKernelGGL((k_cds_march<T, V, ORD, MODE, XT>), dim3(grid), dim3(MARCH_NT), 0, s, n1, n2, n3, r0 / st2, r1 / st2, R0, R1, R2, R3, x, y, b, pout, \
                     xold, partials, done, lg, tiles_x, tiles_y, (int)zchunk, items, st, host, ticket, XV)
  if constexpr (MODE == 4) {
    if (a.march == 1) SIPX_MARCH(1, QUpd<T>, *upd);
    else SIPX_MARCH(2, QUpd<T>, *upd);
  } else {
    if (a.march == 1) SIPX_MARCH(1, NoExtra, NoExtra{});
    else SIPX_MARCH(2, NoExtra, NoExtra{});
  }
#undef SIPX_MARCH
  return true;
}

template <typename T, int MODE>
static void launch_cds(hipStream_t s, long long N, long long r0, long long r1, const T* R, const CdsArgs& a, const T* x, T* y,
                       const T* b, T* pout, T* xold, double* partials, const int* done) {
  if (a.d < 1 || a.d > MAXD) throw std::runtime_error("cds: band count out of range");
  if (r0 < 0 || r1 > N || r0 > r1) throw std::runtime_error("cds: row range outside the matrix");
  int read_bands = a.d;
  if (a.sym) { read_bands = 0; for (int b = 0; b < a.d; ++b) read_bands += a.off[b] >= 0 ? 1 : 0; }
  const double rw = (double)(r1 - r0) * sizeof(T), extra = MODE == 2 ? 4.0 : 2.0;
  const double moved_extra = (MODE == 2 && !xold) ? 3.0 : extra;
  ObsScope obs(MODE == 0 ? KID_CDS_SPMV : (MODE == 1 ? KID_CDS_DOT : KID_CDS_RESID), s, (a.d + extra) * rw, (read_bands + moved_extra) * rw);
  if (try_march<T, MODE>(s, N, r0, r1, R, a, x, y, b, pout, xold, partials, done)) {
    SIPX_HIP(hipGetLastError());
    return;
  }
#define SIPX_CDS(V, D) \
  hipLaunchKernelGGL((k_cds<T, V, D, MODE>), dim3(fit_grid((r1 - r0) / V, SIPX_CG_GRID)), dim3(BLOCK), 0, s, N, r0, r1, R, a, x, y, b, pout, xold, partials, done)
  constexpr int VW = sizeof(T) == 8 ? SIPX_F64_VEC : 4;
  if (N % 4 == 0 && r0 % 4 == 0 && r1 % 4 == 0) {
    switch (a.d) {
      case 1: SIPX_CDS(VW, 1); break;
      case 3: SIPX_CDS(VW, 3); break;
      case 5: SIPX_CDS(VW, 5); break;
      case 7: SIPX_CDS(VW, 7); break;
      default: SIPX_CDS(VW, 0); break;
    }
  } else {
    SIPX_CDS(1, 0);
  }
#undef SIPX_CDS
  SIPX_HIP(hipGetLastError());
}

template <typename T>
void K<T>::spmv(hipStream_t s, const Grid&, long long N, const T* R, const CdsArgs& a, const T* x, T* y) {
  launch_cds<T, 0>(s, N, 0, N, R, a, x, y, nullptr, nullptr, nullptr, nullptr, nullptr);
}
template <typename T>
void K<T>::spmv_dot(hipStream_t s, long long N, long long r0, long long r1, const T* R, const CdsArgs& a, const T* p, T* Ap,
                    double* partials, const CgState<T>* st) {
  launch_cds<T, 1>(s, N, r0, r1, R, a, p, Ap, nullptr, nullptr, nullptr, partials, &st->done);
}
template <typename T>
void K<T>::resid(hipStream_t s, long long N, long long r0, long long r1, const T* R, const CdsArgs& a, const T* x, const T* b,
                 T* r, T* p, T* xold, double* partials) {
  launch_cds<T, 2>(s, N, r0, r1, R, a, x, r, b, p, xold, partials, nullptr);
}

template <typename T, int V>
__device__ __forceinline__ void stencil_rows(const Grid& G, const StencilQ<T>& q, const T* __restrict__ x, long long g,
                                             const Vec<T, V>& xc, T (&acc)[V]) {
  const Coord c = coords(G, g);
#pragma unroll
  for (int k = 0; k < V; ++k) acc[k] = q.w0 * xc.v[k];
#pragma unroll
  for (int dir = 0; dir < 3; ++dir) {
    if (!(q.mask & (1 << dir))) continue;
    const long long st = G.st[dir];
    const int nd = (int)G.n[dir], cd = coord_of(c, dir);
    const Vec<T, V> xm = ldv_u<T, V>(x + g - st), xp = ldv_u<T, V>(x + g + st);
#pragma unroll
    for (int k = 0; k < V; ++k) {
      const int ck = cd + (dir == 0 ? k : 0);
      const T a = xc.v[k] - xm.v[k], b = xc.v[k] - xp.v[k];
      const T t = (ck > 0 ? a : T(0)) + (ck < nd - 1 ? b : T(0));
      acc[k] = acc[k] + q.w[dir] * t;
    }
  }
}

template <typename T, int V, int MODE>
__global__ __launch_bounds__(BLOCK) void k_sq(Grid G, StencilQ<T> q, const T* __restrict__ x, T* __restrict__ y,
                                              const T* __restrict__ b, T* __restrict__ pout, T* __restrict__ xold,
                                              double* __restrict__ partials, const int* __restrict__ done) {
  if (MODE == 1 && *done) return;
  const long long nvec = G.N / V;
  double acc0 = 0, acc1 = 0;
  for (long long vi = (long long)blockIdx.x * BLOCK + threadIdx.x; vi < nvec; vi += (long long)gridDim.x * BLOCK) {
    const long long r = vi * V;
    const Vec<T, V> xv = ldv<T, V>(x + r);
    T s[V];
    stencil_rows<T, V>(G, q, x, r, xv, s);
    Vec<T, V> o;
    if (MODE == 0) {
#pragma unroll
      for (int k = 0; k < V; ++k) o.v[k] = s[k];
      stv_nt<T, V>(y + r, o);
    } else if (MODE == 1) {
#pragma unroll
      for (int k = 0; k < V; ++k) {
        o.v[k] = s[k];
        acc0 += (double)xv.v[k] * (double)s[k];
      }
      stv_nt<T, V>(y + r, o);
    } else {
      const Vec<T, V> bv = ldv<T, V>(b + r);
#pragma unroll
      for (int k = 0; k < V; ++k) {
// ... 198 lines not shown
            const int cl = rem % 3;
            rem /= 3;
            const T ih = S.ih[u], nih = -ih;
            if (cl != 0) val = val + ih * ih;
            if (cl != 2) val = val + nih * nih;
          }
          p.tab[p.ntab++] = S.alpha * val;
        }
      } else {
        int u = -1;
        for (int w = 0; w < S.nblk; ++w)
          if (g.st[S.dir[w]] == (o > 0 ? o : -o)) u = w;
        if (p.ntab + 2 > QP_TAB) return false;
        const T ih = u >= 0 ? S.ih[u] : T(0), nih = -ih;
        t.kind = o > 0 ? 2 : 3;
        t.dir[0] = u >= 0 ? S.dir[u] : 0;
        const T val_on = u >= 0 ? (o > 0 ? T(0) + nih * ih : T(0) + ih * nih) : T(0);
        p.tab[p.ntab++] = S.alpha * val_on;
        p.tab[p.ntab++] = S.alpha * T(0);
      }
    }
    if (nt == 0) continue;
    if (p.nbands == QP_MAXB) return false;
    p.col[p.nbands] = b;
    p.nterms[p.nbands] = nt;
    for (int t = 0; t < nt; ++t) p.t[p.nbands][t] = terms[t];
    p.nbands += 1;
  }
  return true;
}

template <typename T>
void K<T>::q_update(hipStream_t s, const Grid& g, long long r0, long long r1, const CdsArgs& q, const QArgs<T>& a, T* Q) {
  if (a.nsets == 0 || r1 <= r0) return;
  if (r0 < 0 || r1 > g.N) throw std::runtime_error("q_update: row range outside the matrix");
  double touched = 0, survey = 0;
  for (int b = 0; b < q.d; ++b) {
    if (q.sym && q.off[b] < 0) continue;
    bool hit = false;
    for (int si = 0; si < a.nsets; ++si)
      for (int t = 0; t < a.s[si].nband; ++t) {
        if (a.s[si].off[t] != q.off[b]) continue;
        hit = true;
        if (a.s[si].ata) touched += 1;
      }
    touched += hit ? 2 : 0;
  }
  for (int si = 0; si < a.nsets; ++si) survey += 3.0 * a.s[si].nband;
  ObsScope obs(KID_Q_UPDATE, s, survey * (double)(r1 - r0) * sizeof(T), touched * (double)(r1 - r0) * sizeof(T));
  QPlan<T> plan;
  if (env_knobs().q_plan && make_q_plan<T>(g, q, a, plan)) {
    if (plan.nbands == 0) return;
    if (g.n[0] % 4 == 0 && r0 % 4 == 0 && r1 % 4 == 0)
      hipLaunchKernelGGL((k_q_update_plan<T, 4>), dim3(fit_grid((r1 - r0) / 4, NB)), dim3(BLOCK), 0, s, g, r0, r1, plan, Q);
    else
      hipLaunchKernelGGL((k_q_update_plan<T, 1>), dim3(fit_grid(r1 - r0, NB)), dim3(BLOCK), 0, s, g, r0, r1, plan, Q);
    SIPX_HIP(hipGetLastError());
    return;
  }
  if (g.n[0] % 4 == 0 && r0 % 4 == 0 && r1 % 4 == 0)
    hipLaunchKernelGGL((k_q_update<T, 4>), dim3(fit_grid((r1 - r0) / 4, NB)), dim3(BLOCK), 0, s, g, r0, r1, q, a, Q);
  else
    hipLaunchKernelGGL((k_q_update<T, 1>), dim3(fit_grid(r1 - r0, NB)), dim3(BLOCK), 0, s, g, r0, r1, q, a, Q);
  SIPX_HIP(hipGetLastError());
}

template <typename T>
__global__ __launch_bounds__(BLOCK) void k_mirror_bands(long long N, CdsArgs q, T* __restrict__ Q) {
  for (long long r = (long long)blockIdx.x * BLOCK + threadIdx.x; r < N; r += (long long)gridDim.x * BLOCK) {
    for (int b = 0; b < q.d; ++b) {
      const long long o = q.off[b];
      if (o >= 0) continue;
      Q[(long long)b * N + r] = (r + o >= 0) ? Q[(long long)q.partner[b] * N + r + o] : T(0);
    }
  }
}
template <typename T>
void K<T>::mirror_bands(hipStream_t s, long long N, const CdsArgs& q, T* Q) {
  hipLaunchKernelGGL((k_mirror_bands<T>), dim3(NB), dim3(BLOCK), 0, s, N, q, Q);
  SIPX_HIP(hipGetLastError());
}

template <typename T>
__global__ __launch_bounds__(BLOCK) void k_q_update_mk(Grid G, CdsArgs q, MkArgs<T> a, T* __restrict__ Q) {
  const long long N = G.N, Nx = 2 * G.N;
  for (long long g = (long long)blockIdx.x * BLOCK + threadIdx.x; g < Nx; g += (long long)gridDim.x * BLOCK) {
    const int br = g >= N;
    const long long gl = g - (long long)br * N;
    const Coord c = coords(G, gl);
    for (int b = 0; b < q.d; ++b) {
      if (q.sym && q.off[b] < 0) continue;
      const long long cc = g + q.off[b];
      if (cc < 0 || cc >= Nx) continue;
      const int bc = cc >= N;
      const long long o = (cc - (long long)bc * N) - gl;
      T qv = Q[(long long)b * Nx + g];
      for (int si = 0; si < a.nsets; ++si) {
        const MkSet<T>& S = a.s[si];
        const bool pop = S.comp == 3 || (S.comp == 1 && br == 0 && bc == 0) || (S.comp == 2 && br == 1 && bc == 1);
        if (!pop) continue;
        qv = qv + S.alpha * ata_value<T>(G, S.nblk, S.dir, S.ih, o, c);
      }
      Q[(long long)b * Nx + g] = qv;
    }
  }
}
template <typename T>
void K<T>::q_update_mk(hipStream_t s, const Grid& g, const CdsArgs& q, const MkArgs<T>& a, T* Q) {
  if (a.nsets == 0) return;
  hipLaunchKernelGGL((k_q_update_mk<T>), dim3(NB), dim3(BLOCK), 0, s, g, q, a, Q);
  SIPX_HIP(hipGetLastError());
}

template <typename T>
void K<T>::gen_ata(hipStream_t s, const Grid& g, int nblk, const int* dir, const T* ih, int nband, const long long* offs,
                   T* R) {
  GenArgs a;
  a.nblk = nblk;
  a.nband = nband;
  for (int q = 0; q < 3; ++q) a.dir[q] = q < nblk ? dir[q] : 0;
  for (int b = 0; b < nband; ++b) a.off[b] = offs[b];
  hipLaunchKernelGGL((k_gen_ata<T>), dim3(NB), dim3(BLOCK), 0, s, g, a, ih[0], nblk > 1 ? ih[1] : T(0),
                     nblk > 2 ? ih[2] : T(0), R);
  SIPX_HIP(hipGetLastError());
}

__device__ __forceinline__ void publish_ticket(unsigned long long* ticket, unsigned seq, int iter, int done) {
  const unsigned long long v = ((unsigned long long)seq << 32) | ((unsigned long long)(unsigned)iter << 1) | (done ? 1ull : 0ull);
  __hip_atomic_store(ticket, v, __ATOMIC_RELEASE, __HIP_MEMORY_SCOPE_SYSTEM);
}

template <typename T>
__global__ __launch_bounds__(BLOCK) void k_cg_begin(const double* __restrict__ partials, CgState<T>* st,
                                                    CgState<T>* host, int it_outer, T tol_ref, unsigned seq,
                                                    unsigned long long* ticket) {
  const double ss_r = block_sum_partials(partials);
  const double ss_b = block_sum_partials(partials + NB);
  if (threadIdx.x == 0) {
    const T nr0 = (T)sqrt(ss_b), nres = (T)sqrt(ss_r);
    const double cand = jl_max(0.1 * (double)nres / (double)nr0, (double)(T(10) * eps_of<T>()));
    const T tol = (it_outer < 3) ? (T)cand : (T)jl_min(cand, (double)tol_ref);
    st->tol = tol;
    st->tol_ref = tol;
    st->nr0 = nr0;
    st->ss = ss_r;
    st->rr = (T)ss_r;
    st->gamma = st->alpha = st->beta = T(0);
    st->res_last = T(0);
    st->iters = 0;
    st->flag = -1;
    st->done = 0;
    st->it_outer = it_outer;
    st->seq = seq;
    if (nr0 == T(0)) {
      st->flag = -9;
      st->done = 1;
    } else if (nres / nr0 <= tol) {
      st->flag = 0;
      st->done = 1;
      st->iters = 1;
    }
    *host = *st;
    publish_ticket(ticket, seq, 0, st->done);
  }
}
template <typename T>
// ... 79 lines not shown
    } else {
      st->beta = beta;
    }
    st->rr = rr;
    *host = *st;
    publish_ticket(ticket, st->seq, st->iters, conv ? 1 : 0);
  }
  if (conv) return;
  const long long nvec = N / V;
  for (long long vi = (long long)blockIdx.x * BLOCK + threadIdx.x; vi < nvec; vi += (long long)gridDim.x * BLOCK) {
    Vec<T, V> pv = ldv<T, V>(p + vi * V);
    const Vec<T, V> rv = ldv<T, V>(r + vi * V);
#pragma unroll
    for (int k = 0; k < V; ++k) pv.v[k] = rv.v[k] + beta * pv.v[k];
    stv<T, V>(p + vi * V, pv);
  }
  for (long long j = (long long)blockIdx.x * BLOCK + threadIdx.x; j < hlo + hhi; j += (long long)gridDim.x * BLOCK) {
    const long long i = j < hlo ? j - hlo : N + (j - hlo);
    p[i] = r[i] + beta * p[i];
  }
}
template <typename T>
void K<T>::cg_update_p(hipStream_t s, long long N, T* p, const T* r, const double* partials, CgState<T>* st,
                       CgState<T>* host, unsigned long long* ticket, long long hlo, long long hhi) {
  ObsScope obs(KID_CG_P, s, 3.0 * (double)N * sizeof(T));
  if (N % 4 == 0 && aligned16(p, r))
    hipLaunchKernelGGL((k_cg_update_p<T, 4>), dim3(fit_grid(N / 4, NB)), dim3(BLOCK), 0, s, N, p, r, partials, st, host, ticket, hlo, hhi);
  else
    hipLaunchKernelGGL((k_cg_update_p<T, 1>), dim3(fit_grid(N, NB)), dim3(BLOCK), 0, s, N, p, r, partials, st, host, ticket, hlo, hhi);
  SIPX_HIP(hipGetLastError());
}

template <typename T, int V, int D>
__global__ __launch_bounds__(BLOCK) void k_cds_fused(long long N, const T* __restrict__ R, CdsArgs a, const T* __restrict__ r,
                                                     const T* __restrict__ p_old, T* __restrict__ p_new, T* __restrict__ Ap,
                                                     double* __restrict__ partials, CgState<T>* __restrict__ st,
                                                     CgState<T>* __restrict__ host, unsigned long long* ticket) {
  if (st->done) return;
  const double ss = block_sum_partials(partials + NB);
  const T rr = (T)ss;
  const T res = (T)sqrt(ss) / st->nr0;
  const bool conv = res <= st->tol;
  const T beta = rr / st->gamma;
  if (blockIdx.x == 0 && threadIdx.x == 0) {
    st->ss = ss;
    st->res_last = res;
    if (conv) {
      st->flag = 0;
      st->done = 1;
    } else {
      st->beta = beta;
    }
    st->rr = rr;
    *host = *st;
    publish_ticket(ticket, st->seq, st->iters, conv ? 1 : 0);
  }
  if (conv) return;
  const LoadFused<T, V> xl{r, p_old, beta};
  const long long nvec = N / V;
  double acc0 = 0;
  for (long long vi = (long long)blockIdx.x * BLOCK + threadIdx.x; vi < nvec; vi += (long long)gridDim.x * BLOCK) {
    const long long row = vi * V;
    T s[V];
    cds_rows<T, V, D>(N, R, a, xl, row, s);
    const Vec<T, V> pv = xl(row);
    Vec<T, V> o;
#pragma unroll
    for (int k = 0; k < V; ++k) {
      o.v[k] = s[k];
      acc0 += (double)pv.v[k] * (double)s[k];
    }
    stv<T, V>(p_new + row, pv);
    stv_nt<T, V>(Ap + row, o);
  }
  double acc[1] = {acc0};
  block_reduce_store<1>(acc, partials, 0);
}
template <typename T>
void K<T>::spmv_fused(hipStream_t s, long long N, const T* R, const CdsArgs& a, const T* r, const T* p_old, T* p_new, T* Ap,
                      double* partials, CgState<T>* st, CgState<T>* host, unsigned long long* ticket) {
  if (a.d < 1 || a.d > MAXD) throw std::runtime_error("cds: band count out of range");
  int read_bands = a.d;
  if (a.sym) { read_bands = 0; for (int b = 0; b < a.d; ++b) read_bands += a.off[b] >= 0 ? 1 : 0; }
  ObsScope obs(KID_CDS_FUSED, s, (a.d + 4.0) * (double)N * sizeof(T), (read_bands + 4.0) * (double)N * sizeof(T));
  if (try_march<T, 3>(s, N, 0, N, R, a, r, Ap, p_old, p_new, nullptr, partials, nullptr, st, host, ticket)) {
    SIPX_HIP(hipGetLastError());
    return;
  }
#define SIPX_CDSF(V, D) \
  hipLaunchKernelGGL((k_cds_fused<T, V, D>), dim3(fit_grid(N / V, SIPX_CG_GRID)), dim3(BLOCK), 0, s, N, R, a, r, p_old, p_new, Ap, partials, st, host, ticket)
  constexpr int VW = sizeof(T) == 8 ? SIPX_F64_VEC : 4;
  if (N % 4 == 0) {
    switch (a.d) {
      case 1: SIPX_CDSF(VW, 1); break;
      case 3: SIPX_CDSF(VW, 3); break;
      case 5: SIPX_CDSF(VW, 5); break;
      case 7: SIPX_CDSF(VW, 7); break;
      default: SIPX_CDSF(VW, 0); break;
    }
  } else {
    SIPX_CDSF(1, 0);
  }
#undef SIPX_CDSF
  SIPX_HIP(hipGetLastError());
}

template <typename T>
bool K<T>::resid_qupdate(hipStream_t s, const Grid& g, long long N, const T* R_old, T* R_new, const CdsArgs& a, const QArgs<T>& qa, const T* x,
                         const T* b, T* r, T* p, T* xold, double* partials) {
  if (!a.march || !a.sym || a.d != 7 || qa.nsets == 0) return false;
  for (int i = 0; i < qa.nsets; ++i)
    if (qa.s[i].ata) return false;
  QUpd<T> u;
  if (!make_q_plan<T>(g, a, qa, u.plan)) return false;
  for (int q = 0; q < 4; ++q) {
    u.qn[q] = R_new + (long long)a.mb[q] * N;
    u.pb[q] = -1;
    for (int b = 0; b < u.plan.nbands; ++b)
      if (u.plan.col[b] == a.mb[q]) u.pb[q] = b;
  }
  u.G = g;
  const double rw = (double)N * sizeof(T);
  ObsScope obs(KID_CDS_RESID, s, (a.d + 4.0) * rw + 3.0 * 4.0 * rw, (4.0 + 4.0) * rw + 4.0 * rw);
  return try_march<T, 4>(s, N, 0, N, R_old, a, x, r, b, p, xold, partials, nullptr, nullptr, nullptr, nullptr, &u);
}

__global__ __launch_bounds__(BLOCK) void k_fin_sum(const double* __restrict__ partials, double* __restrict__ out_dev,
                                                   double* __restrict__ out_host, unsigned* __restrict__ ticket,
                                                   unsigned long long* __restrict__ word, unsigned long long seq) {
  const double s = block_sum_partials(partials + (long long)blockIdx.x * NB);
  if (threadIdx.x == 0) {
    if (out_dev) out_dev[blockIdx.x] = s;
    if (out_host) out_host[blockIdx.x] = s;
    if (word) {
      __threadfence_system();
      const unsigned t = __hip_atomic_fetch_add(ticket, 1u, __ATOMIC_ACQ_REL, __HIP_MEMORY_SCOPE_AGENT);
      if (t == gridDim.x - 1) {
        __hip_atomic_store(ticket, 0u, __ATOMIC_RELAXED, __HIP_MEMORY_SCOPE_AGENT);
        __threadfence_system();
        __hip_atomic_store(word, seq, __ATOMIC_RELEASE, __HIP_MEMORY_SCOPE_SYSTEM);
      }
    }
  }
}
template <typename T>
void K<T>::fin_sum(hipStream_t s, const double* partials, int nslots, double* out_dev, double* out_host, unsigned* ticket,
                   unsigned long long* word, unsigned long long seq) {
  ObsScope obs(KID_FIN_SUM, s, (double)nslots * NB * sizeof(double));
  hipLaunchKernelGGL(k_fin_sum, dim3(nslots), dim3(BLOCK), 0, s, partials, out_dev, out_host, ticket, word, seq);
  SIPX_HIP(hipGetLastError());
}

__global__ __launch_bounds__(BLOCK) void k_copy_f64(const double* __restrict__ src, double* __restrict__ dst, int n) {
  for (int i = threadIdx.x; i < n; i += BLOCK) dst[i] = src[i];
}
template <typename T>
void K<T>::copy_f64(hipStream_t s, const double* src, double* dst, int n) {
  hipLaunchKernelGGL(k_copy_f64, dim3(1), dim3(BLOCK), 0, s, src, dst, n);
  SIPX_HIP(hipGetLastError());
}

#define SIPX_INST(T)                                                                                                  \
  template void K<T>::spmv(hipStream_t, const Grid&, long long, const T*, const CdsArgs&, const T*, T*);             \
  template void K<T>::spmv_dot(hipStream_t, long long, long long, long long, const T*, const CdsArgs&, const T*, T*, \
                               double*, const CgState<T>*);                                                           \
  template void K<T>::spmv_fused(hipStream_t, long long, const T*, const CdsArgs&, const T*, const T*, T*, T*, double*, \
                                 CgState<T>*, CgState<T>*, unsigned long long*);                                      \
  template void K<T>::resid(hipStream_t, long long, long long, long long, const T*, const CdsArgs&, const T*, const T*, T*, \
                            T*, T*, double*);                                                                         \
  template bool K<T>::resid_qupdate(hipStream_t, const Grid&, long long, const T*, T*, const CdsArgs&, const QArgs<T>&, const T*, \
                                    const T*, T*, T*, T*, double*);                                                   \
  template void K<T>::q_axpy(hipStream_t, long long, T*, const T*, T);                                               \
  template void K<T>::q_update_mk(hipStream_t, const Grid&, const CdsArgs&, const MkArgs<T>&, T*);                    \
  template void K<T>::mirror_bands(hipStream_t, long long, const CdsArgs&, T*);                                       \
  template void K<T>::sq_spmv(hipStream_t, const Grid&, const StencilQ<T>&, const T*, T*);                           \
  template void K<T>::sq_spmv_dot(hipStream_t, const Grid&, const StencilQ<T>&, const T*, T*, double*,               \
                                  const CgState<T>*);                                                                 \
  template void K<T>::sq_resid(hipStream_t, const Grid&, const StencilQ<T>&, const T*, const T*, T*, T*, T*, double*); \
  template void K<T>::q_update(hipStream_t, const Grid&, long long, long long, const CdsArgs&, const QArgs<T>&, T*);  \
  template void K<T>::gen_ata(hipStream_t, const Grid&, int, const int*, const T*, int, const long long*, T*);       \
  template void K<T>::cg_begin(hipStream_t, double*, CgState<T>*, CgState<T>*, int, T, unsigned, unsigned long long*);  \
  template void K<T>::cg_update_xr(hipStream_t, long long, const T*, T*, const T*, T*, const T*, const T*, double*, CgState<T>*, \
                                   CgState<T>*, int, unsigned long long*, long long, long long);                     \
  template void K<T>::cg_update_p(hipStream_t, long long, T*, const T*, const double*, CgState<T>*, CgState<T>*,     \
                                  unsigned long long*, long long, long long);                                        \
  template void K<T>::fin_sum(hipStream_t, const double*, int, double*, double*, unsigned*, unsigned long long*, unsigned long long); \
  template void K<T>::copy_f64(hipStream_t, const double*, double*, int);
SIPX_INST(float)
SIPX_INST(double)

}
```

### setintersectionprojection.jl_amd/csrc/sipx_common.h

```cpp
#pragma once
#include <hip/hip_runtime.h>
#include <stdint.h>
#include <cstdio>

namespace sipx {

constexpr int BLOCK = 256;
constexpr int NB = 2048;
constexpr int NB_7 = 1792;
inline int fit_grid(long long nvec, int cap) {
  const long long need = (nvec + BLOCK - 1) / BLOCK;
  return (int)(need < 1 ? 1 : (need < cap ? need : cap));
}
template <typename... P>
inline bool aligned16(const P*... p) {
  return (((reinterpret_cast<uintptr_t>(p) & 15u) == 0) && ...);
}
inline int launch_blocks(int per_cu) {
  static const int cus = [] {
    int dev = 0, n = 0;
    if (hipGetDevice(&dev) != hipSuccess || hipDeviceGetAttribute(&n, hipDeviceAttributeMultiprocessorCount, dev) != hipSuccess || n <= 0)
      n = 256;
    return n;
  }();
  const int g = per_cu * cus;
  return g < 256 ? 256 : (g > NB_7 ? NB_7 : g);
}
constexpr int MAXD = 32;
constexpr int MAX_SETS = 16;
constexpr int YL_SLOTS = 13;
constexpr int L1_K = 8;
#define SIPX_SOLVE_SLOTS 64
#define SIPX_MAX_WORLD 64
constexpr int GATHER_HDR = 8;
constexpr int PREP_SLOTS = 3 + 2 * L1_K;
template <typename T>
constexpr int fast_hdr() { return ((PREP_SLOTS + 4) * 8 / (int)sizeof(T) + 3) / 4 * 4; }
constexpr int SAMPLE_BINS = 1024;
constexpr int SAMPLE_MBITS = 7;

enum KernelId {
  KID_CDS_SPMV = 0, KID_CDS_DOT, KID_CDS_RESID, KID_CDS_FUSED, KID_SQ_SPMV, KID_SQ_DOT, KID_SQ_RESID, KID_CG_BEGIN, KID_CG_XR, KID_CG_P,
  KID_Q_UPDATE, KID_FIN_SUM, KID_RHS, KID_YL, KID_YL_MULTI, KID_ADJ_NORM, KID_LOG3, KID_PASS_FIRST, KID_PASS_LEAN, KID_PASS_PROBE,
  KID_PASS_COMPACT, KID_PASS_DIST, KID_PASS_STORE, KID_PASS_MULTI, KID_SLOT_SUMS, KID_DECIDE, KID_SAMPLE, KID_L1_SOLVE, KID_GATHER,
  KID_PS_RESCALE, KID_CARD, KID_EXT, KID_BB_RULE, KID_OTHER, KID_COUNT
};
inline const char* kernel_name(int k) {
  static const char* const names[KID_COUNT] = {
      "k_cds<MODE=0>", "k_cds<MODE=1>", "k_cds<MODE=2>", "k_cds_fused", "k_sq<MODE=0>", "k_sq<MODE=1>", "k_sq<MODE=2>", "k_cg_begin",
      "k_cg_update_xr", "k_cg_update_p", "k_q_update", "k_fin_sum", "k_rhs", "k_yl", "k_yl_multi", "k_adj_norm", "k_log3",
      "k_pass<M_FIRST>", "k_pass<M_LEAN>", "k_pass<M_PROBE>", "k_pass<M_COMPACT>", "k_pass<M_DIST>", "k_pass<M_STORE>", "k_pass_multi",
      "k_slot_sums", "k_decide", "k_sample", "k_l1_solve", "k_gather_pack/unpack", "k_ps_rescale", "k_card_*", "ext_proj (library-backed)",
      "k_bb_rule", "other"};
  return (k >= 0 && k < KID_COUNT) ? names[k] : "?";
}
struct LaunchObserver {
  void* user;
  void (*begin)(void* user, int kid, hipStream_t s, double bytes_survey, double bytes_moved);
  void (*end)(void* user, int kid, hipStream_t s);
};
const LaunchObserver*& launch_observer();

struct EnvKnobs {
  int cds_march = 1;
  long long cds_march_zchunk = 0;
  long long multi_zchunk = 0;
  int rhs_march = 1;
  long long rhs_march_zchunk = 0;
  int trace_kernels = 0;
  int trace_searches = 0;
  int mark_stride = 0;
  int q_plan = 1;
};
const EnvKnobs& env_knobs();
void refresh_env_knobs();
long long*& alloc_tally();
struct ObsScope {
  const LaunchObserver* o;
  int kid;
  hipStream_t s;
  ObsScope(int kid_, hipStream_t s_, double bytes_survey, double bytes_moved = -1.0) : o(launch_observer()), kid(kid_), s(s_) {
    if (env_knobs().trace_kernels) fprintf(stderr, "[sipx trace] %s\n", kernel_name(kid));
    if (o) o->begin(o->user, kid, s, bytes_survey, bytes_moved < 0 ? bytes_survey : bytes_moved);
  }
  ~ObsScope() {
    if (o) o->end(o->user, kid, s);
    if (env_knobs().trace_kernels) {
      (void)hipStreamSynchronize(s);
      fprintf(stderr, "[sipx trace]   done\n");
    }
  }
  ObsScope(const ObsScope&) = delete;
  ObsScope& operator=(const ObsScope&) = delete;
};

enum { SL_RPRI = 0, SL_DY = 1, SL_HL = 2, SL_HH = 3, SL_LH = 4, SL_DL = 5, SL_GG = 6, SL_GL = 7,
       SL_FE = 8, SL_SS = 9, SL_OBJ = 10, SL_EVO = 11, SL_XX = 12,
       SL_ADJ = 13 , SL_FE2 = 14, SL_SS2 = 15  };
constexpr int SET_SLOTS = 16;

enum { F_FEAS = 1, F_BB = 2, F_FIRST = 4, F_NOSPEC = 8 ,
       F_STORE_DY = 16  };

enum { PX_BOUNDS = 0, PX_BOUNDS_VEC = 1, PX_L1 = 2, PX_L2 = 3, PX_ANNULUS = 4, PX_CARD = 5, PX_PROX_L1 = 6,
       PX_EXT = 8,
       PX_DIST = 100 };

struct Grid {
  long long n[3];
  long long N;
  long long st[3];
  unsigned m1 = 0, s1 = 0, m2 = 0, s2 = 0;
  long long e0 = 0, e1 = -1, s0 = 0;
  void set_fast_div() {
    auto magic = [](long long d, unsigned& m, unsigned& sh) {
      m = 0; sh = 0;
      if (d < 2 || d >= (1ll << 31)) return;
      int l = 0;
      while ((1ll << l) < d) ++l;
      const unsigned long long q = ((unsigned long long)1 << (31 + l)) / (unsigned long long)d + 1ull;
      m = (unsigned)q;
      sh = (unsigned)(l - 1);
    };
    magic(n[0], m1, s1);
    magic(n[1], m2, s2);
  }
};

inline long long range_len(const Grid& g) { return (g.e1 < 0 ? g.N : g.e1) - g.e0; }

struct CdsArgs {
  int d;
  long long off[MAXD];
  int sym = 0;
  int partner[MAXD] = {};
  int march = 0;
  int mb[4] = {0, 0, 0, 0};
  long long gn[3] = {0, 0, 0};
};

template <typename T>
struct StencilQ {
  T w0, w[3];
  int mask;
};

template <typename T>
struct ProjScalars {
  double asum;
  double sumsq;
  T vmax;
  T vmin;
  int need;
  T theta;
  T scale;
  int fill;
  double t[L1_K];
  double lo, hi;
  int refine;
  int rounds_used;
  double theta_prev;
  unsigned long long n_compact;
  double spec_lo, spec_hi;
  double s_above, c_above;
  double hw;
  int spec_ok, spec_overflow;
  double dbg[4];
  T tau;
  long long quota;
  long long* cidx;
  double c_lo, c_hi;
  double br_tl, br_Sl, br_Cl, br_th, br_Sh, br_Ch;
  T tau_prev;
  double red[PREP_SLOTS];
  double ovf;
  double mm[2 * SIPX_MAX_WORLD];
  int gather_overflow;
  int lean;
  double coop_hi[2][SIPX_SOLVE_SLOTS], coop_lo[2][SIPX_SOLVE_SLOTS], coop_c[2][SIPX_SOLVE_SLOTS];
  unsigned coop_arrive, coop_finish, coop_abort;
  unsigned long long hist[SAMPLE_BINS];
  unsigned pass_ticket;
  unsigned samp_ticket;
  int rescaled, resc_bad;
  int want_sample;
  int sampled;
  int dbg_sampled;
  double samp_theta;
  double samp_bias;
  int samp_bias_ok;
  double samp_lo, samp_hi, samp_c;
};

struct ChainHooks {
  int world = 1, rank = 0;
  void* user = nullptr;
  void (*allreduce_sum)(void* user, double* buf, size_t count, hipStream_t s) = nullptr;
  void (*allgather)(void* user, void* buf, size_t chunk, int dtype_is_f64, hipStream_t s) = nullptr;
  void* gbuf = nullptr;
  long long gcap = 0;
  long long fcap = 0;
};

struct SampleCtl {
  int enable = 0;
  long long runs = 0;
  int* host_want = nullptr;
  int* host_ovf = nullptr;
  unsigned* verdict = nullptr;
  unsigned seq = 0;
  int lean_done = 0;
  int lean_known = 0;
  long long compact_cap = 0;
};

template <typename T>
struct SetArgs {
  T *y, *l, *dy, *lh0, *y0, *s0, *l0;
  T *yo, *lo;
  T* v;
  const T *x, *m, *xold, *lb, *ub;
// ... 135 lines not shown
struct MkArgs {
  int nsets;
  MkSet<T> s[MAX_SETS];
};

template <typename T>
struct QSet {
  T alpha;
  const T* ata;
  int nblk;
  int dir[3];
  T ih[3];
  int nband;
  long long off[9];
};
template <typename T>
struct QArgs {
  int nsets;
  QSet<T> s[MAX_SETS];
};

template <typename T>
struct RhsSet {
  const T *y, *l;
  T rho;
  int nblk;
  int dir[3];
  T ih[3];
};
template <typename T>
struct RhsArgs {
  int nsets;
  RhsSet<T> s[MAX_SETS];
};

template <typename T>
struct CgState {
  double ss;
  T rr;
  T gamma, alpha, beta;
  T nr0, tol, res_last;
  int done, flag, iters;
  T tol_ref;
  int it_outer;
  unsigned seq;
};

template <typename T>
struct K {
  static void spmv(hipStream_t s, const Grid& g, long long N, const T* R, const CdsArgs& a, const T* x, T* y);
  static void spmv_dot(hipStream_t s, long long N, long long r0, long long r1, const T* R, const CdsArgs& a, const T* p, T* Ap,
                       double* partials, const CgState<T>* st);
  static void resid(hipStream_t s, long long N, long long r0, long long r1, const T* R, const CdsArgs& a, const T* x, const T* b,
                    T* r, T* p, T* xold, double* partials);
  static bool resid_qupdate(hipStream_t s, const Grid& g, long long N, const T* R_old, T* R_new, const CdsArgs& a, const QArgs<T>& qa,
                            const T* x, const T* b, T* r, T* p, T* xold, double* partials);
  static void spmv_fused(hipStream_t s, long long N, const T* R, const CdsArgs& a, const T* r, const T* p_old, T* p_new, T* Ap,
                         double* partials, CgState<T>* st, CgState<T>* host, unsigned long long* ticket);
  static void sq_spmv(hipStream_t s, const Grid& g, const StencilQ<T>& q, const T* x, T* y);
  static void sq_spmv_dot(hipStream_t s, const Grid& g, const StencilQ<T>& q, const T* p, T* Ap, double* partials,
                          const CgState<T>* st);
  static void sq_resid(hipStream_t s, const Grid& g, const StencilQ<T>& q, const T* x, const T* b, T* r, T* p, T* xold,
                       double* partials);
  static void q_axpy(hipStream_t s, long long N, T* Qband, const T* Aband, T alpha);
  static void q_update(hipStream_t s, const Grid& g, long long r0, long long r1, const CdsArgs& q, const QArgs<T>& a, T* Q);
  static void gen_ata(hipStream_t s, const Grid& g, int nblk, const int* dir, const T* ih, int nband,
                      const long long* offs, T* R);
  static void cg_begin(hipStream_t s, double* partials, CgState<T>* st, CgState<T>* host, int it_outer, T tol_ref,
                       unsigned seq, unsigned long long* ticket);
  static void cg_update_xr(hipStream_t s, long long N, const T* x_in, T* x, const T* r_in, T* r, const T* p, const T* Ap, double* partials,
                           CgState<T>* st, CgState<T>* host, int iter, unsigned long long* ticket, long long hlo = 0,
                           long long hhi = 0);
  static void cg_update_p(hipStream_t s, long long N, T* p, const T* r, const double* partials, CgState<T>* st,
                          CgState<T>* host, unsigned long long* ticket, long long hlo = 0, long long hhi = 0);
  static void rhs_compose(hipStream_t s, const Grid& g, const RhsArgs<T>& a, T* rhs, int accumulate);
  static void yl(hipStream_t s, const Grid& g, const SetArgs<T>& a, double* partials);
  static void adj_norm(hipStream_t s, const Grid& g, const SetArgs<T>& a, double* partials);
  static bool yl_multi(hipStream_t s, const Grid& g, const MultiArgs<T>& a, bool probe_only = false);
  static void fwd(hipStream_t s, const Grid& g, int nblk, const int* dir, const T* ih, const T* x, T* out);
  static void adj(hipStream_t s, const Grid& g, int nblk, const int* dir, const T* ih, const T* v, T* out);
  static void log3(hipStream_t s, long long N, const T* x, const T* m, const T* xold, double* partials);
  static void q_update_mk(hipStream_t s, const Grid& g, const CdsArgs& q, const MkArgs<T>& a, T* Q);
  static void mirror_bands(hipStream_t s, long long N, const CdsArgs& q, T* Q);
  static void sum_uv(hipStream_t s, long long N, const T* u, const T* v, T* w);
  static void csr_spmv(hipStream_t s, long long M, const long long* rowptr, const long long* col, const T* val, const T* x, T* out);
  static void csc_adj_rhs(hipStream_t s, long long N, const long long* colptr, const long long* row, const T* val, const T* y,
                          const T* l, T rho, T* out, int accumulate);
  static void csc_adj_norm(hipStream_t s, long long N, const long long* colptr, const long long* row, const T* val, const T* dy,
                           double* partials);
  static void rows_pack(hipStream_t s, const Grid& g, int dir, long long nrows, const T* pad, T* rows);
  static void rows_unpack(hipStream_t s, const Grid& g, int dir, long long nrows, const T* rows, T* pad);
  static void fin_sum(hipStream_t s, const double* partials, int nslots, double* out_dev, double* out_host, unsigned* ticket = nullptr,
                      unsigned long long* word = nullptr, unsigned long long seq = 0);
  static void copy_f64(hipStream_t s, const double* src, double* dst, int n);
  static void ps_rescale(hipStream_t s, ProjScalars<T>* ps, double factor);
  static void proj_scalars_set(hipStream_t s, const Grid& g, const SetArgs<T>& a, int v_is_s, ProjScalars<T>* ps,
                               double* partials, T* maxpart, T* compact, long long true_len, SampleCtl ctl = SampleCtl(),
                               const ChainHooks* hooks = nullptr);
  static void spec_sums_pack(hipStream_t s, const SpecPackArgs<T>& A);
  static void spec_finish(hipStream_t s, SpecFinishArgs<T>& A);
  static void ps_rescale_multi(hipStream_t s, const RescaleMulti<T>& A);
  static void sample_multi(int stage, hipStream_t s, const Grid& g, const SampleMulti<T>& A, long long runs, const ChainHooks* hk);
  static void lean_multi(hipStream_t s, const Grid& g, const LeanMulti<T>& m);
  static void pass_multi(int mode, hipStream_t s, const Grid& g, const LeanMulti<T>& m, int v_is_s);
  static void search_tail(int stage, hipStream_t s, const SetArgs<T>& a, ProjScalars<T>* ps, double* partials, T* maxpart, T* compact,
                          long long true_len, SampleCtl ctl, double* reg);
  static void proj_scalars_stage(int stage, hipStream_t s, const Grid& g, const SetArgs<T>& a, int v_is_s, ProjScalars<T>* ps,
                                 double* partials, T* maxpart, T* compact, long long true_len, SampleCtl ctl, const ChainHooks* hooks,
                                 double* reg, T* gseg0, long long chunk);
  static void proj_scalars_arr(hipStream_t s, long long len, const T* v, int prox, T pmin, T pmax, ProjScalars<T>* ps,
                               double* partials, T* maxpart, T* compact, long long true_len);
  static void proj_scalars_arr_slab(hipStream_t s, long long len, const T* v, int prox, T pmin, T pmax, ProjScalars<T>* ps,
                                    double* partials, T* maxpart, T* compact, long long true_len, const ChainHooks* hooks,
                                    long long compact_len, int* host_ovf);
  static void proj_dist_set(hipStream_t s, const Grid& g, const SetArgs<T>& a, int v_is_s, const ProjScalars<T>* ps,
                            double* dst);
  static void ps_init(hipStream_t s, ProjScalars<T>* ps, long long* cidx);
  static void store_v(hipStream_t s, const Grid& g, const SetArgs<T>& a, int v_is_s, T* out);
};

template <typename T>
void proj_dist_grid(hipStream_t s, const Grid& g, int nblk, const int* dir, long long len, const T* v, int prox, T plo,
                    T phi, const T* lb, const T* ub, const ProjScalars<T>* ps, double* partials);
template <typename T>
void proj_apply_grid(hipStream_t s, const Grid& g, int nblk, const int* dir, long long len, T* v, int prox, T plo,
                     T phi, const T* lb, const T* ub, const ProjScalars<T>* ps);

template <typename T>
void prox_l2s_dev(hipStream_t s, long long n, T* x, const T* m, T rho);

template <typename T>
void resample_nn(hipStream_t s, const long long* nc, const long long* nf, const T* in, T* out);
template <typename T>
void resample_nn_rows(hipStream_t s, const long long* nc, const long long* nf, int nblk, const int* dir, int b, long long cstride,
                      long long e0, long long e1, const T* in, T* out);
template <typename T>
void resample_nn_padded(hipStream_t s, const long long* nc, const long long* nf, const long long* cc, const long long* cf, long long e0,
                        long long e1, const T* in, T* out);

#define SIPX_HIP(expr)                                                                       \
  do {                                                                                       \
    hipError_t _e = (expr);                                                                  \
    if (_e != hipSuccess) throw std::runtime_error(std::string(#expr) + ": " + hipGetErrorString(_e)); \
  } while (0)

}
```

Measured before the change: 777.8.

## Replace Q band storage with a 27-class boundary table in the z-marching SpMV

When the 7-band symmetric Q on a 3-D grid is constant within each of the 27 boundary classes, the engine builds a small table of band values per class and checks it on the device against the assembled bands. The marching CG kernel then reads band coefficients from that table in shared memory instead of streaming four full-length band arrays. Rho updates modify only the table, and the bands are written back lazily when Q is read out. This removes most of the matrix memory traffic per CG iteration, at the cost of a one-time check with a host sync, fallbacks when no update plan exists, and extra per-element class arithmetic. The boundary mask is also simplified to precomputed booleans.

```diff
diff --git a/setintersectionprojection.jl_amd/csrc/engine.cpp b/setintersectionprojection.jl_amd/csrc/engine.cpp
--- a/setintersectionprojection.jl_amd/csrc/engine.cpp
+++ b/setintersectionprojection.jl_amd/csrc/engine.cpp
@@ -35,6 +35,7 @@
   k.rhs_march = (int)num("SIPX_RHS_MARCH", 1);
   k.rhs_march_zchunk = num("SIPX_RHS_MARCH_ZCHUNK", 0);
   k.q_plan = (int)num("SIPX_Q_PLAN", 1);
+  k.q_table = (int)num("SIPX_Q_TABLE", 1);
   k.mark_stride = (int)std::max<long long>(0, num("SIPX_MARK_STRIDE", 0));
   k.trace_searches = (int)num("SIPX_TRACE_SEARCHES", 0);
   k.trace_kernels = (int)num("SIPX_TRACE_KERNELS", 0);
@@ -385,7 +386,7 @@
     if (loose_owned_) { dfree(loose_v_); dfree(loose_w_); }
     (void)hipStreamSynchronize(stream_);
     for (auto& s : sets_) free_set(s);
-    for (void* p : {(void*)xr_base_[0], (void*)xr_base_[1], (void*)xr_base_[2], (void*)w_base_, (void*)rhs_, (void*)m_base_, (void*)r_base_, (void*)p_base_, (void*)p2_base_, (void*)Ap_, (void*)Q_, (void*)Q2_,
+    for (void* p : {(void*)xr_base_[0], (void*)xr_base_[1], (void*)xr_base_[2], (void*)w_base_, (void*)rhs_, (void*)m_base_, (void*)r_base_, (void*)p_base_, (void*)p2_base_, (void*)Ap_, (void*)Q_, (void*)Q2_, (void*)qtab_,
                     (void*)scr_v_, (void*)scr_c_, (void*)scr_i_, (void*)scr_w_, (void*)part_cg_, (void*)part_tmp_, (void*)part_sets_,
                     (void*)maxpart_, (void*)cg_dev_, (void*)gbuf_, (void*)stage_, (void*)sstage_, (void*)fbuf_, (void*)agree_buf_})
       dfree(p);
@@ -915,6 +916,7 @@
 
     assemble_Q();
     if (q_fused_ && !stencil_q_ && !comm_ && cds_.march != 0) Q2_ = dalloc<T>((size_t)Nx_ * cds_.d);
+    build_q_table();
     {
       const char* ln = std::getenv("SIPX_RANK_LANE");
       lane_set_ = -1;
@@ -1034,6 +1036,7 @@
     mark_step_[0] = mark_step_[1] = 0;
     run_ = Run();
     assemble_Q();
+    build_q_table();
     initial_feasibility(feasibility_initial);
   }
 
@@ -2458,12 +2461,57 @@
         return;
       }
     }
-    K<T>::q_update(stream_, G_, qr0_, qr1_, cds_, a, Q_);
+    q_apply(a);
   }
   void flush_q_pending() {
     if (!q_pending_) return;
     q_pending_ = false;
-    K<T>::q_update(stream_, G_, qr0_, qr1_, cds_, q_pending_args_, Q_);
+    q_apply(q_pending_args_);
+  }
+  void q_apply(const QArgs<T>& a) {
+    if (cds_.qtab) {
+      if (K<T>::qtab_update(stream_, G_, cds_, a, qtab_)) {
+        q_stale_ = q_stale_ || a.nsets > 0;
+        return;
+      }
+      ensure_q_bands();
+      cds_.qtab = nullptr;
+      qtab_reason_ = "an update without a plan";
+    }
+    K<T>::q_update(stream_, G_, qr0_, qr1_, cds_, a, Q_);
+  }
+  void ensure_q_bands() {
+    if (!q_stale_) return;
+    K<T>::qtab_write_bands(stream_, Nx_, cds_, qtab_, Q_);
+    q_stale_ = false;
+  }
+  void build_q_table() {
+    cds_.qtab = nullptr;
+    q_stale_ = false;
+    const char* why = nullptr;
+    if (!env_knobs().q_table) why = "SIPX_Q_TABLE=0";
+    else if (stencil_q_) why = "stencil Q";
+    else if (q_fused_) why = "SIPX_Q_FUSED";
+    else if (mk_) why = "Minkowski";
+    else if (comm_) why = "sharded";
+    else if (!cds_.march || !cds_.sym || cds_.d != 7) why = "not the 7-band matrix of a 3-D grid";
+    else if (qr0_ != 0 || qr1_ != Nx_ || !K<T>::march_applies(Nx_, cds_)) why = "the z-marching product does not apply";
+    if (why) {
+      qtab_reason_ = why;
+      return;
+    }
+    if (!qtab_) qtab_ = dalloc<T>(QT_N + 8);
+    int* ok = (int*)(qtab_ + QT_N);
+    K<T>::qtab_build(stream_, Nx_, cds_, Q_, qtab_, ok);
+    int h = 0;
+    SIPX_HIP(hipMemcpyAsync(&h, ok, sizeof(int), hipMemcpyDeviceToHost, stream_));
+    SIPX_HIP(hipStreamSynchronize(stream_));
+    if (!h) {
+      qtab_reason_ = "Q is not constant on the boundary classes";
+      return;
+    }
+    cds_.qtab = qtab_;
+    qtab_reason_ = "";
   }
 
   void warm_start_from(EngineBase* coarse_base) override {
@@ -2916,6 +2964,7 @@
     if (Q && stencil_q_) throw std::runtime_error("stencil Q mode stores no bands (use sipx_apply_Q)");
     if (Q && comm_ && comm_->world > 1) throw std::runtime_error("a sharded context maintains its slab of Q only");
     flush_q_pending();
+    if (Q) ensure_q_bands();
     if (Q && cds_.sym) {
       K<T>::mirror_bands(stream_, Nx_, cds_, Q_);
       SIPX_HIP(hipStreamSynchronize(stream_));
@@ -3007,6 +3056,7 @@
       o += ", \"comm_selftest\": \"" + t + "\"";
     }
     o += ", \"lane_set\": " + std::to_string(lane_set_);
+    o += std::string(", \"q_table\": {\"on\": ") + (cds_.qtab ? "true" : "false") + ", \"reason\": \"" + qtab_reason_ + "\"}";
     o += ", \"batched_searches\": {\"searches\": " + std::to_string(batch_searches_) + ", \"fallbacks\": " + std::to_string(batch_fallbacks_) + "}";
     long long rc[6] = {0, 0, 0, 0, 0, 0};
     for (const auto& st : sets_) {
@@ -3442,6 +3492,8 @@
   }
 
   void assemble_Q() {
+    cds_.qtab = nullptr;
+    q_stale_ = false;
     if (stencil_q_) {
       for (auto& s : sets_)
         if (s.ata) throw std::runtime_error("stencil Q mode needs descriptor-generated AtA for every set (pass ata_R = NULL)");
@@ -3472,7 +3524,7 @@
     QArgs<T> a;
     a.nsets = 0;
     for (int i = 0; i < p_n_; ++i) push_qset(a, sets_[i], rho_[i]);
-    K<T>::q_update(stream_, G_, qr0_, qr1_, cds_, a, Q_);
+    q_apply(a);
   }
 
   void mk_q_update(const std::vector<T>& alpha) {
@@ -3499,7 +3551,7 @@
     if (s.ata_off.size() > 9) throw std::runtime_error("more than 9 bands in one set's AtA are not supported");
     for (long long o : s.ata_off) (void)q_col(o);
     if (a.nsets == MAX_SETS) {
-      K<T>::q_update(stream_, G_, qr0_, qr1_, cds_, a, Q_);
+      q_apply(a);
       a.nsets = 0;
     }
     QSet<T>& q = a.s[a.nsets++];
@@ -3882,6 +3934,9 @@
   hipEvent_t ev_sums_ = nullptr, ev_cgb_ = nullptr;
   bool sums_pending_ = false, defer_sums_ = false;
   bool q_fused_ = false, q_pending_ = false, q_defer_ = false;
+  T* qtab_ = nullptr;
+  bool q_stale_ = false;
+  std::string qtab_reason_ = "not built";
   QArgs<T> q_pending_args_;
   T* Q2_ = nullptr;
   long long dev_bytes_ = 0;
diff --git a/setintersectionprojection.jl_amd/csrc/kernels_cds.hip b/setintersectionprojection.jl_amd/csrc/kernels_cds.hip
--- a/setintersectionprojection.jl_amd/csrc/kernels_cds.hip
+++ b/setintersectionprojection.jl_amd/csrc/kernels_cds.hip
@@ -170,6 +170,14 @@
   Grid G;
 };
 struct NoExtra {};
+template <typename T>
+struct QTab {
+  const T* tab;
+};
+template <typename X>
+struct IsQTab { static constexpr bool value = false; };
+template <typename T>
+struct IsQTab<QTab<T>> { static constexpr bool value = true; };
 template <typename T>
 __device__ __forceinline__ T q_upd_val(const QUpd<T>& u, const T* __restrict__ tab, int role, const Coord& c, T qv) {
   const int b = u.pb[role];
@@ -198,14 +206,20 @@
 template <typename T>
 __device__ __forceinline__ T q_upd_val(const NoExtra&, const T*, int, const Coord&, T qv) { return qv; }
 template <typename T>
+__device__ __forceinline__ T q_upd_val(const QTab<T>&, const T*, int, const Coord&, T qv) { return qv; }
+template <typename T>
 __device__ __forceinline__ void load_plan_tab(const QUpd<T>& u, T* tab) {
   for (int i = threadIdx.x; i < u.plan.ntab; i += blockDim.x) tab[i] = u.plan.tab[i];
 }
 template <typename T>
 __device__ __forceinline__ void load_plan_tab(const NoExtra&, T*) {}
 template <typename T>
+__device__ __forceinline__ void load_plan_tab(const QTab<T>&, T*) {}
+template <typename T>
 __device__ __forceinline__ const Grid& extra_grid(const QUpd<T>& u) { return u.G; }
 __device__ __forceinline__ Grid extra_grid(const NoExtra&) { return Grid{}; }
+template <typename T>
+__device__ __forceinline__ Grid extra_grid(const QTab<T>&) { return Grid{}; }
 template <typename T, int V>
 __device__ __forceinline__ void store_bands(const QUpd<T>& u, long long r, const Vec<T, V>& r0, const Vec<T, V>& r1, const Vec<T, V>& r2,
                                             const Vec<T, V>& r3) {
@@ -216,6 +230,24 @@
 }
 template <typename T, int V>
 __device__ __forceinline__ void store_bands(const NoExtra&, long long, const Vec<T, V>&, const Vec<T, V>&, const Vec<T, V>&, const Vec<T, V>&) {}
+template <typename T, int V>
+__device__ __forceinline__ void store_bands(const QTab<T>&, long long, const Vec<T, V>&, const Vec<T, V>&, const Vec<T, V>&, const Vec<T, V>&) {}
+template <typename T>
+__device__ __forceinline__ void load_class_tab(const QTab<T>& u, T* tab) {
+  for (int i = threadIdx.x; i < QT_N; i += blockDim.x) tab[i] = u.tab[i];
+}
+template <typename X, typename T>
+__device__ __forceinline__ void load_class_tab(const X&, T*) {}
+__device__ __forceinline__ int line_class(long long c, long long n) { return c == 0 ? 0 : (c == n - 1 ? 2 : 1); }
+template <typename T, int V>
+__device__ __forceinline__ Vec<T, V> tab_row(const T* tab, int role, int cyz, long long i0, long long n1) {
+  const T* e = tab + 27 * role + cyz;
+  const T first = e[0], mid = e[1], last = e[2];
+  Vec<T, V> v;
+#pragma unroll
+  for (int k = 0; k < V; ++k) v.v[k] = i0 + k == 0 ? first : (i0 + k == n1 - 1 ? last : mid);
+  return v;
+}
 __device__ __forceinline__ void publish_ticket(unsigned long long* ticket, unsigned seq, int iter, int done);
 constexpr int MARCH_NT = 512;
 template <typename T, int V, int ORD, int MODE, typename X>
@@ -227,6 +259,7 @@
                                                         long long items, CgState<T>* __restrict__ st, CgState<T>* __restrict__ host,
                                                         unsigned long long* ticket, X extra) {
   constexpr bool UPD = MODE == 4;
+  constexpr bool TAB = IsQTab<X>::value;
   if (MODE == 1 && *done) return;
   T beta = T(0);
   if (MODE == 3) {
@@ -256,10 +289,15 @@
     return v;
   };
   auto ldx1 = [&](long long at) -> T { return MODE == 3 ? x[at] + beta * b[at] : x[at]; };
-  __shared__ T sx[2][V][MARCH_NT], sr[2][V][MARCH_NT];
+  __shared__ T sx[2][V][MARCH_NT], sr[TAB ? 1 : 2][TAB ? 1 : V][TAB ? 1 : MARCH_NT];
   __shared__ T qtab[UPD ? QP_TAB : 1];
+  __shared__ T ctab[TAB ? QT_N : 1];
   if (UPD) {
     load_plan_tab<T>(extra, qtab);
+    __syncthreads();
+  }
+  if (TAB) {
+    load_class_tab(extra, ctab);
     __syncthreads();
   }
   const int tid = threadIdx.x, LX = 1 << lgLX, tx = tid & (LX - 1), ty = tid >> lgLX, TY = MARCH_NT >> lgLX;
@@ -278,7 +316,9 @@
     if (active) {
       xm = ldx(st2 * (k0 - 1) + go);
       x0 = ldx(st2 * k0 + go);
-      if (k0 > 0) {
+      if (k0 > 0 && TAB) {
+        rzm = tab_row<T, V>(ctab, 3, 3 * line_class(j, n2) + 9 * line_class(k0 - 1, n3), i0, n1);
+      } else if (k0 > 0) {
         rzm = ldv<T, V>(R3 + st2 * (k0 - 1) + go);
         if (UPD) {
 #pragma unroll
@@ -290,12 +330,21 @@
       const int par = (int)(kz & 1);
       const long long pz = st2 * kz;
       Vec<T, V> xp = zerov<T, V>(), r0 = xp, r1 = xp, r2 = xp, r3 = xp, bv = xp;
+      const int cz = TAB ? line_class(kz, n3) : 0, cyz = TAB ? 3 * line_class(j, n2) + 9 * cz : 0;
+      const int cyz_up = !TAB ? 0 : (j > 0 ? 3 * line_class(j - 1, n2) + 9 * cz : 3 * line_class(n2 - 1, n2) + 9 * line_class(kz - 1, n3));
       if (active) {
         xp = ldx(pz + st2 + go);
-        r0 = ldv_nt<T, V>(R0 + pz + go);
-        r1 = ldv_nt<T, V>(R1 + pz + go);
-        r2 = ldv_nt<T, V>(R2 + pz + go);
-        r3 = ldv_nt<T, V>(R3 + pz + go);
+        if constexpr (TAB) {
+          r0 = tab_row<T, V>(ctab, 0, cyz, i0, n1);
+          r1 = tab_row<T, V>(ctab, 1, cyz, i0, n1);
+          r2 = tab_row<T, V>(ctab, 2, cyz, i0, n1);
+          r3 = tab_row<T, V>(ctab, 3, cyz, i0, n1);
+        } else {
+          r0 = ldv_nt<T, V>(R0 + pz + go);
+          r1 = ldv_nt<T, V>(R1 + pz + go);
+          r2 = ldv_nt<T, V>(R2 + pz + go);
+          r3 = ldv_nt<T, V>(R3 + pz + go);
+        }
         if (MODE == 2 || MODE == 4) bv = ldv<T, V>(b + pz + go);
         if (UPD) {
 #pragma unroll
@@ -309,13 +358,18 @@
         }
       }
 #pragma unroll
-      for (int k = 0; k < V; ++k) { sx[par][k][tid] = x0.v[k]; sr[par][k][tid] = r2.v[k]; }
-      T xl = __shfl_up(x0.v[V - 1], 1, 64), xr = __shfl_down(x0.v[0], 1, 64), rl = __shfl_up(r1.v[V - 1], 1, 64);
+      for (int k = 0; k < V; ++k) {
+        sx[par][k][tid] = x0.v[k];
+        if constexpr (!TAB) sr[par][k][tid] = r2.v[k];
+      }
+      T xl = __shfl_up(x0.v[V - 1], 1, 64), xr = __shfl_down(x0.v[0], 1, 64), rl = TAB ? T(0) : __shfl_up(r1.v[V - 1], 1, 64);
       const long long r = pz + go;
+      if (TAB && r > 0)
+        rl = i0 > 0 ? ctab[27 + line_class(i0 - 1, n1) + cyz] : ctab[27 + line_class(n1 - 1, n1) + cyz_up];
       if (active) {
         if (tx == 0 || (tid & 63) == 0) {
           xl = ldx1(r - 1);
-          rl = r > 0 ? R1[r - 1] : T(0);
+          if (!TAB) rl = r > 0 ? R1[r - 1] : T(0);
           if (UPD && r > 0) rl = q_upd_val<T>(extra, qtab, 1, coords(extra_grid(extra), r - 1), rl);
         }
         if (tx == LX - 1 || (tid & 63) == 63) xr = ldx1(r + V);
@@ -323,12 +377,16 @@
       __syncthreads();
       if (active) {
         Vec<T, V> xu = zerov<T, V>(), xd = xu, ru = xu;
+        if (TAB && r - st1 >= 0) ru = tab_row<T, V>(ctab, 2, cyz_up, i0, n1);
         if (ty > 0) {
 #pragma unroll
-          for (int k = 0; k < V; ++k) { xu.v[k] = sx[par][k][tid - LX]; ru.v[k] = sr[par][k][tid - LX]; }
+          for (int k = 0; k < V; ++k) {
+            xu.v[k] = sx[par][k][tid - LX];
+            if constexpr (!TAB) ru.v[k] = sr[par][k][tid - LX];
+          }
         } else {
           xu = ldx(r - st1);
-          if (r - st1 >= 0) {
+          if (!TAB && r - st1 >= 0) {
             ru = ldv<T, V>(R2 + r - st1);
             if (UPD) {
 #pragma unroll
@@ -342,20 +400,19 @@
         } else {
           xd = ldx(r + st1);
         }
+        const bool up = r >= st1, down = r + st1 < N, below = r >= st2, above = r + st2 < N, first = r == 0, last = r + V == N;
         Vec<T, V> o4;
 #pragma unroll
         for (int k = 0; k < V; ++k) {
-          const long long rr = r + k;
           const T rv[7] = {r0.v[k], k == 0 ? rl : r1.v[k - 1], r1.v[k], ru.v[k], r2.v[k], rzm.v[k], r3.v[k]};
           const T xv[7] = {x0.v[k], k == 0 ? xl : x0.v[k - 1], k == V - 1 ? xr : x0.v[k + 1], xu.v[k], xd.v[k], xm.v[k], xp.v[k]};
-          const long long co[7] = {0, -1, 1, -st1, st1, -st2, st2};
+          const bool in[7] = {true, k > 0 || !first, k < V - 1 || !last, up, down, below, above};
           T acc = T(0);
 #pragma unroll
           for (int q = 0; q < 7; ++q) {
             const int role = march_role(ORD, q);
             const T t = acc + rv[role] * xv[role];
-            const long long c = rr + co[role];
-            acc = (c >= 0 && c < N) ? t : acc;
+            acc = in[role] ? t : acc;
           }
           o4.v[k] = acc;
         }
@@ -400,10 +457,12 @@
   }
 }
 
-template <typename T, int MODE>
-static bool try_march(hipStream_t s, long long N, long long r0, long long r1, const T* R, const CdsArgs& a, const T* x, T* y, const T* b,
-                      T* pout, T* xold, double* partials, const int* done, CgState<T>* st = nullptr, CgState<T>* host = nullptr,
-                      unsigned long long* ticket = nullptr, const QUpd<T>* upd = nullptr) {
+struct MarchGeom {
+  int lg, tiles_x, tiles_y, zchunk, grid;
+  long long items;
+};
+template <typename T>
+static bool march_geom(long long N, long long r0, long long r1, const CdsArgs& a, MarchGeom& m) {
   const int sw = env_knobs().cds_march;
   const long long zc_env = env_knobs().cds_march_zchunk;
   if (sw == 0 || !a.march || !a.sym || a.d != 7) return false;
@@ -422,17 +481,40 @@
   if (zchunk > planes) zchunk = planes;
   const long long nchunks = (planes + zchunk - 1) / zchunk, items = tiles * nchunks;
   if (items < 384 && sw != 2) return false;
-  const int grid = (int)(items < NB ? items : NB);
+  m = MarchGeom{lg, tiles_x, tiles_y, (int)zchunk, (int)(items < NB ? items : NB), items};
+  return true;
+}
+template <typename T>
+bool K<T>::march_applies(long long N, const CdsArgs& a) {
+  MarchGeom m;
+  return march_geom<T>(N, 0, N, a, m);
+}
+
+template <typename T, int MODE>
+static bool try_march(hipStream_t s, long long N, long long r0, long long r1, const T* R, const CdsArgs& a, const T* x, T* y, const T* b,
+                      T* pout, T* xold, double* partials, const int* done, CgState<T>* st = nullptr, CgState<T>* host = nullptr,
+                      unsigned long long* ticket = nullptr, const QUpd<T>* upd = nullptr) {
+  MarchGeom m;
+  if (!march_geom<T>(N, r0, r1, a, m)) return false;
+  constexpr int V = sizeof(T) == 8 ? 2 : 4;
+  const long long n1 = a.gn[0], n2 = a.gn[1], n3 = a.gn[2], st2 = n1 * n2;
   const T *R0 = R + (long long)a.mb[0] * N, *R1 = R + (long long)a.mb[1] * N, *R2 = R + (long long)a.mb[2] * N, *R3 = R + (long long)a.mb[3] * N;
 #define SIPX_MARCH(ORD, XT, XV)                                                                                                      \
-  hipLaunchKernelGGL((k_cds_march<T, V, ORD, MODE, XT>), dim3(grid), dim3(MARCH_NT), 0, s, n1, n2, n3, r0 / st2, r1 / st2, R0, R1, R2, R3, x, y, b, pout, \
-                     xold, partials, done, lg, tiles_x, tiles_y, (int)zchunk, items, st, host, ticket, XV)
+  hipLaunchKernelGGL((k_cds_march<T, V, ORD, MODE, XT>), dim3(m.grid), dim3(MARCH_NT), 0, s, n1, n2, n3, r0 / st2, r1 / st2, R0, R1, R2, R3, x, y, b, \
+                     pout, xold, partials, done, m.lg, m.tiles_x, m.tiles_y, m.zchunk, m.items, st, host, ticket, XV)
   if constexpr (MODE == 4) {
     if (a.march == 1) SIPX_MARCH(1, QUpd<T>, *upd);
     else SIPX_MARCH(2, QUpd<T>, *upd);
   } else {
-    if (a.march == 1) SIPX_MARCH(1, NoExtra, NoExtra{});
-    else SIPX_MARCH(2, NoExtra, NoExtra{});
+    if (a.qtab) {
+      const QTab<T> tab{(const T*)a.qtab};
+      if (a.march == 1) SIPX_MARCH(1, QTab<T>, tab);
+      else SIPX_MARCH(2, QTab<T>, tab);
+    } else if (a.march == 1) {
+      SIPX_MARCH(1, NoExtra, NoExtra{});
+    } else {
+      SIPX_MARCH(2, NoExtra, NoExtra{});
+    }
   }
 #undef SIPX_MARCH
   return true;
@@ -445,6 +527,7 @@
   if (r0 < 0 || r1 > N || r0 > r1) throw std::runtime_error("cds: row range outside the matrix");
   int read_bands = a.d;
   if (a.sym) { read_bands = 0; for (int b = 0; b < a.d; ++b) read_bands += a.off[b] >= 0 ? 1 : 0; }
+  if (a.qtab) read_bands = 0;
   const double rw = (double)(r1 - r0) * sizeof(T), extra = MODE == 2 ? 4.0 : 2.0;
   const double moved_extra = (MODE == 2 && !xold) ? 3.0 : extra;
   ObsScope obs(MODE == 0 ? KID_CDS_SPMV : (MODE == 1 ? KID_CDS_DOT : KID_CDS_RESID), s, (a.d + extra) * rw, (read_bands + moved_extra) * rw);
@@ -452,6 +535,7 @@
     SIPX_HIP(hipGetLastError());
     return;
   }
+  if (a.qtab) throw std::runtime_error("internal: Q's class table is in use but the z-marching product does not apply");
 #define SIPX_CDS(V, D) \
   hipLaunchKernelGGL((k_cds<T, V, D, MODE>), dim3(fit_grid((r1 - r0) / V, SIPX_CG_GRID)), dim3(BLOCK), 0, s, N, r0, r1, R, a, x, y, b, pout, xold, partials, done)
   constexpr int VW = sizeof(T) == 8 ? SIPX_F64_VEC : 4;
@@ -816,6 +900,119 @@
 }
 
 template <typename T>
+__global__ __launch_bounds__(BLOCK) void k_qtab_seed(long long n1, long long n2, long long n3, CdsArgs q, const T* __restrict__ Q,
+                                                     T* __restrict__ tab, int* __restrict__ ok) {
+  const int t = threadIdx.x;
+  if (t == 0) *ok = 1;
+  if (t >= QT_N) return;
+  const int role = t / 27, c = t % 27, cl[3] = {c % 3, (c / 3) % 3, c / 9};
+  const long long n[3] = {n1, n2, n3};
+  long long at[3];
+  bool exists = true;
+  for (int d = 0; d < 3; ++d) {
+    at[d] = cl[d] == 0 ? 0 : (cl[d] == 2 ? n[d] - 1 : 1);
+    exists = exists && line_class(at[d], n[d]) == cl[d];
+  }
+  tab[t] = exists ? Q[(long long)q.mb[role] * n1 * n2 * n3 + at[0] + n1 * (at[1] + n2 * at[2])] : T(0);
+}
+template <typename T>
+__device__ __forceinline__ bool same_bits(T a, T b) {
+  if constexpr (sizeof(T) == 8) return __double_as_longlong(a) == __double_as_longlong(b);
+  else return __float_as_uint(a) == __float_as_uint(b);
+}
+template <typename T>
+__global__ __launch_bounds__(BLOCK) void k_qtab_check(long long n1, long long n2, long long n3, CdsArgs q, const T* __restrict__ Q,
+                                                      const T* __restrict__ tab, int* __restrict__ ok) {
+  __shared__ T ctab[QT_N];
+  for (int i = threadIdx.x; i < QT_N; i += BLOCK) ctab[i] = tab[i];
+  __syncthreads();
+  const long long N = n1 * n2 * n3;
+  bool bad = false;
+  for (long long row = blockIdx.x; row < n2 * n3; row += gridDim.x) {
+    const long long k = row / n2, j = row - k * n2;
+    const int cyz = 3 * line_class(j, n2) + 9 * line_class(k, n3);
+    for (long long i = threadIdx.x; i < n1; i += BLOCK) {
+      const int c = line_class(i, n1) + cyz;
+      for (int role = 0; role < 4; ++role) bad |= !same_bits(Q[(long long)q.mb[role] * N + row * n1 + i], ctab[27 * role + c]);
+    }
+  }
+  if (bad) *ok = 0;
+}
+template <typename T>
+void K<T>::qtab_build(hipStream_t s, long long N, const CdsArgs& q, const T* Q, T* tab, int* ok) {
+  const long long n1 = q.gn[0], n2 = q.gn[1], n3 = q.gn[2];
+  if (n1 * n2 * n3 != N) throw std::runtime_error("qtab_build: the grid is not the matrix's");
+  hipLaunchKernelGGL((k_qtab_seed<T>), dim3(1), dim3(BLOCK), 0, s, n1, n2, n3, q, Q, tab, ok);
+  SIPX_HIP(hipGetLastError());
+  hipLaunchKernelGGL((k_qtab_check<T>), dim3(NB), dim3(BLOCK), 0, s, n1, n2, n3, q, Q, tab, ok);
+  SIPX_HIP(hipGetLastError());
+}
+template <typename T>
+__global__ __launch_bounds__(BLOCK) void k_qtab_bands(long long n1, long long n2, long long n3, CdsArgs q, const T* __restrict__ tab,
+                                                      T* __restrict__ Q) {
+  __shared__ T ctab[QT_N];
+  for (int i = threadIdx.x; i < QT_N; i += BLOCK) ctab[i] = tab[i];
+  __syncthreads();
+  const long long N = n1 * n2 * n3;
+  for (long long row = blockIdx.x; row < n2 * n3; row += gridDim.x) {
+    const long long k = row / n2, j = row - k * n2;
+    const int cyz = 3 * line_class(j, n2) + 9 * line_class(k, n3);
+    for (long long i = threadIdx.x; i < n1; i += BLOCK) {
+      const int c = line_class(i, n1) + cyz;
+      for (int role = 0; role < 4; ++role) Q[(long long)q.mb[role] * N + row * n1 + i] = ctab[27 * role + c];
+    }
+  }
+}
+template <typename T>
+void K<T>::qtab_write_bands(hipStream_t s, long long N, const CdsArgs& q, const T* tab, T* Q) {
+  const long long n1 = q.gn[0], n2 = q.gn[1], n3 = q.gn[2];
+  if (n1 * n2 * n3 != N) throw std::runtime_error("qtab_write_bands: the grid is not the matrix's");
+  ObsScope obs(KID_Q_UPDATE, s, 4.0 * (double)N * sizeof(T), 4.0 * (double)N * sizeof(T));
+  hipLaunchKernelGGL((k_qtab_bands<T>), dim3(NB), dim3(BLOCK), 0, s, n1, n2, n3, q, tab, Q);
+  SIPX_HIP(hipGetLastError());
+}
+template <typename T>
+__global__ __launch_bounds__(BLOCK) void k_qtab_update(QPlan<T> p, CdsArgs q, T* __restrict__ tab) {
+  const int t = threadIdx.x;
+  if (t >= QT_N) return;
+  const int role = t / 27, c = t % 27, cx = c % 3, cy = (c / 3) % 3, cz = c / 9;
+  int b = -1;
+  for (int u = 0; u < p.nbands; ++u)
+    if (p.col[u] == q.mb[role]) b = u;
+  if (b < 0) return;
+  T qv = tab[t];
+  for (int ti = 0; ti < p.nterms[b]; ++ti) {
+    const QPlanTerm& m = p.t[b][ti];
+    if (m.kind == 0) {
+      qv = qv + p.tab[m.tab];
+    } else if (m.kind == 1) {
+      int idx = 0, m3 = 1;
+      for (int u = 0; u < m.nblk; ++u) {
+        const int d = m.dir[u];
+        idx += (d == 0 ? cx : (d == 1 ? cy : cz)) * m3;
+        m3 *= 3;
+      }
+      qv = qv + p.tab[m.tab + idx];
+    } else {
+      const int d = m.dir[0], cl = d == 0 ? cx : (d == 1 ? cy : cz);
+      qv = qv + (cl != (m.kind == 2 ? 2 : 0) ? p.tab[m.tab] : p.tab[m.tab + 1]);
+    }
+  }
+  tab[t] = qv;
+}
+template <typename T>
+bool K<T>::qtab_update(hipStream_t s, const Grid& g, const CdsArgs& q, const QArgs<T>& a, T* tab) {
+  if (a.nsets == 0) return true;
+  QPlan<T> plan;
+  if (!env_knobs().q_plan || !make_q_plan<T>(g, q, a, plan)) return false;
+  if (plan.nbands == 0) return true;
+  ObsScope obs(KID_Q_UPDATE, s, 2.0 * QT_N * sizeof(T), 2.0 * QT_N * sizeof(T));
+  hipLaunchKernelGGL((k_qtab_update<T>), dim3(1), dim3(BLOCK), 0, s, plan, q, tab);
+  SIPX_HIP(hipGetLastError());
+  return true;
+}
+
+template <typename T>
 __global__ __launch_bounds__(BLOCK) void k_q_update_mk(Grid G, CdsArgs q, MkArgs<T> a, T* __restrict__ Q) {
   const long long N = G.N, Nx = 2 * G.N;
   for (long long g = (long long)blockIdx.x * BLOCK + threadIdx.x; g < Nx; g += (long long)gridDim.x * BLOCK) {
@@ -1061,11 +1258,13 @@
   if (a.d < 1 || a.d > MAXD) throw std::runtime_error("cds: band count out of range");
   int read_bands = a.d;
   if (a.sym) { read_bands = 0; for (int b = 0; b < a.d; ++b) read_bands += a.off[b] >= 0 ? 1 : 0; }
+  if (a.qtab) read_bands = 0;
   ObsScope obs(KID_CDS_FUSED, s, (a.d + 4.0) * (double)N * sizeof(T), (read_bands + 4.0) * (double)N * sizeof(T));
   if (try_march<T, 3>(s, N, 0, N, R, a, r, Ap, p_old, p_new, nullptr, partials, nullptr, st, host, ticket)) {
     SIPX_HIP(hipGetLastError());
     return;
   }
+  if (a.qtab) throw std::runtime_error("internal: Q's class table is in use but the z-marching product does not apply");
 #define SIPX_CDSF(V, D) \
   hipLaunchKernelGGL((k_cds_fused<T, V, D>), dim3(fit_grid(N / V, SIPX_CG_GRID)), dim3(BLOCK), 0, s, N, R, a, r, p_old, p_new, Ap, partials, st, host, ticket)
   constexpr int VW = sizeof(T) == 8 ? SIPX_F64_VEC : 4;
@@ -1152,6 +1351,10 @@
   template void K<T>::q_axpy(hipStream_t, long long, T*, const T*, T);                                               \
   template void K<T>::q_update_mk(hipStream_t, const Grid&, const CdsArgs&, const MkArgs<T>&, T*);                    \
   template void K<T>::mirror_bands(hipStream_t, long long, const CdsArgs&, T*);                                       \
+  template bool K<T>::march_applies(long long, const CdsArgs&);                                                      \
+  template void K<T>::qtab_build(hipStream_t, long long, const CdsArgs&, const T*, T*, int*);                         \
+  template bool K<T>::qtab_update(hipStream_t, const Grid&, const CdsArgs&, const QArgs<T>&, T*);                     \
+  template void K<T>::qtab_write_bands(hipStream_t, long long, const CdsArgs&, const T*, T*);                         \
   template void K<T>::sq_spmv(hipStream_t, const Grid&, const StencilQ<T>&, const T*, T*);                           \
   template void K<T>::sq_spmv_dot(hipStream_t, const Grid&, const StencilQ<T>&, const T*, T*, double*,               \
                                   const CgState<T>*);                                                                 \
diff --git a/setintersectionprojection.jl_amd/csrc/sipx_common.h b/setintersectionprojection.jl_amd/csrc/sipx_common.h
--- a/setintersectionprojection.jl_amd/csrc/sipx_common.h
+++ b/setintersectionprojection.jl_amd/csrc/sipx_common.h
@@ -28,6 +28,7 @@
 }
 constexpr int MAXD = 32;
 constexpr int MAX_SETS = 16;
+constexpr int QT_N = 4 * 27;
 constexpr int YL_SLOTS = 13;
 constexpr int L1_K = 8;
 #define SIPX_SOLVE_SLOTS 64
@@ -71,6 +72,7 @@
   int trace_searches = 0;
   int mark_stride = 0;
   int q_plan = 1;
+  int q_table = 1;
 };
 const EnvKnobs& env_knobs();
 void refresh_env_knobs();
@@ -137,6 +139,7 @@
   int march = 0;
   int mb[4] = {0, 0, 0, 0};
   long long gn[3] = {0, 0, 0};
+  const void* qtab = nullptr;
 };
 
 template <typename T>
@@ -438,6 +441,10 @@
   static void log3(hipStream_t s, long long N, const T* x, const T* m, const T* xold, double* partials);
   static void q_update_mk(hipStream_t s, const Grid& g, const CdsArgs& q, const MkArgs<T>& a, T* Q);
   static void mirror_bands(hipStream_t s, long long N, const CdsArgs& q, T* Q);
+  static bool march_applies(long long N, const CdsArgs& a);
+  static void qtab_build(hipStream_t s, long long N, const CdsArgs& q, const T* Q, T* tab, int* ok);
+  static bool qtab_update(hipStream_t s, const Grid& g, const CdsArgs& q, const QArgs<T>& a, T* tab);
+  static void qtab_write_bands(hipStream_t s, long long N, const CdsArgs& q, const T* tab, T* Q);
   static void sum_uv(hipStream_t s, long long N, const T* u, const T* v, T* w);
   static void csr_spmv(hipStream_t s, long long M, const long long* rowptr, const long long* col, const T* val, const T* x, T* out);
   static void csc_adj_rhs(hipStream_t s, long long N, const long long* colptr, const long long* row, const T* val, const T* y,
```

Result: faster. 886.5 (median of 6 runs) (+14.0%).
